# tkeskita/smoothMesh

Measured on AMD Instinct MI355X. Metric: mesh-points smoothed/sec/node (100 iters) + achieved HBM GB/s vs roofline, higher is better.
Workload: dtype f64

## Files before the change

### include/smgpu.h

```cpp
#ifndef SMGPU_H
#define SMGPU_H

#include <stddef.h>
#include <stdint.h>

#ifdef __cplusplus
extern "C" {
#endif

typedef struct smgpu_handle smgpu_handle;

typedef struct smgpu_mesh_desc {
    int32_t nPoints, nCells, nFaces, nInternalFaces;
    const double* points;
    const int32_t* faceOffsets;
    const int32_t* facePoints;
    const int32_t* owner;
    const int32_t* neighbour;
    const uint8_t* isInternalPoint;
    const uint8_t* isSmoothingSurfacePoint;
    int32_t device;
    void* stream;
    int32_t useCallerStream;
} smgpu_mesh_desc;
// ... 123 lines not shown
    void* localFlags;
} smgpu_push_desc;
int smgpu_halo_set_push(smgpu_handle* h, const smgpu_push_desc* d);
int smgpu_push_alloc(int32_t device, size_t bytes, void** ptr, void* ipcHandle64);
int smgpu_push_open(int32_t device, const void* ipcHandle64, void** ptr);
int smgpu_push_close(void* ptr);
int smgpu_push_free(void* ptr);

int smgpu_halo_set_exchange_stream(smgpu_handle* h, int32_t useExchangeStream, void* exchangeStream);
int smgpu_get_stream(smgpu_handle* h, void** stream);
int smgpu_halo_set_stats_history(smgpu_handle* h, void* history, int32_t capacity);
int smgpu_iter_begin(smgpu_handle* h);
int smgpu_iter_interior(smgpu_handle* h);
int smgpu_iter_mid(smgpu_handle* h);
int smgpu_iter_ahead(smgpu_handle* h);
int smgpu_iter_end(smgpu_handle* h);

typedef struct smgpu_layer_desc {
    int32_t nPatches;
    const int32_t* patchStart;
    const int32_t* patchSize;
    const uint8_t* patchKind;
    const uint8_t* isLayerPatch;
    double layerMaxBlendingFraction;
    double layerEdgeLength;
    double layerExpansionRatio;
    int32_t minLayers, maxLayers;
} smgpu_layer_desc;
int smgpu_set_layers(smgpu_handle* h, const smgpu_layer_desc* d, int32_t* enabled);

enum { SMGPU_LAYERS_HOPS_SWEEP = 0, SMGPU_LAYERS_NORMALS_ACCUMULATE = 1, SMGPU_LAYERS_NORMALS_FINISH = 2,
       SMGPU_LAYERS_PROPAGATE_SWEEP = 3, SMGPU_LAYERS_FINISH = 4 };
enum { SMGPU_LAYERS_F_HOPS = 0,
       SMGPU_LAYERS_F_NORMALS_COUNT = 1,
       SMGPU_LAYERS_F_NORMALS = 2 };
#define SMGPU_HALO_L_DOUBLES 14
#define SMGPU_HALO_L_LAYERS 6
int smgpu_halo_l_doubles(smgpu_handle* h, int32_t* doublesPerSlot);
int smgpu_layers_begin(smgpu_handle* h, const smgpu_layer_desc* d, int32_t* enabled, int32_t* maxIter);
int smgpu_layers_step(smgpu_handle* h, int32_t step, int32_t arg);
int smgpu_layers_shared(smgpu_handle* h, int32_t field, int32_t set, double* values);

typedef struct smgpu_boundary_desc {
    int32_t nPatches;
    const int32_t* patchStart;
    const int32_t* patchSize;
    const uint8_t* patchKind;
    const uint8_t* isSmoothingPatch;
    int32_t nInitEdgePoints;   const double* initEdgePoints;
    int32_t nInitEdges;        const int32_t* initEdges;
    int32_t nTargetEdgePoints; const double* targetEdgePoints;
    int32_t nTargetEdges;      const int32_t* targetEdges;
    int32_t nSurfacePoints;    const double* surfacePoints;
    int32_t nSurfaceTriangles; const int32_t* surfaceTriangles;
    const int32_t* isCornerPointIO;
    const int32_t* isFeatureEdgePointIO;
    double distanceTolerance;
    double internalSmoothingBlendingFraction;
} smgpu_boundary_desc;
typedef struct smgpu_boundary_info {
    int32_t enabled;
    int32_t nCornerPoints, nFeatureEdgePoints, nSmoothingSurfacePoints, nFrozenSurfacePoints;
    int32_t nTargetEdgeStrings;
} smgpu_boundary_info;
int smgpu_set_boundary_smoothing(smgpu_handle* h, const smgpu_boundary_desc* d, smgpu_boundary_info* info);
enum { SMGPU_BOUNDARY_HOPS_SWEEP = 0, SMGPU_BOUNDARY_TABLES = 1, SMGPU_BOUNDARY_NORMALS_ACCUMULATE = 2, SMGPU_BOUNDARY_NORMALS_FINISH = 3 };
enum { SMGPU_BOUNDARY_F_HOPS = 0,
       SMGPU_BOUNDARY_F_NORMALS_COUNT = 1 };
int smgpu_boundary_stats(smgpu_handle* h, double* minEdgeLength, double* boundingBox );
int smgpu_boundary_begin(smgpu_handle* h, const smgpu_boundary_desc* d, double minEdgeLengthGlobal, double perimeterGlobal,
                         smgpu_boundary_info* info);
int smgpu_boundary_step(smgpu_handle* h, int32_t step);
int smgpu_boundary_shared(smgpu_handle* h, int32_t field, int32_t set, double* values);
int smgpu_get_boundary_classification(smgpu_handle* h, int32_t* isCornerPoint, int32_t* isFeatureEdgePoint);
int smgpu_debug_edge_strings(int32_t nPoints, int32_t nEdges, const int32_t* edges, int32_t* strings, int32_t* nStrings);
int smgpu_debug_find_line(smgpu_handle* h, int32_t n, const double* segments, double* hitPoints, int32_t* hit);

int smgpu_set_device_share(smgpu_handle* h, int32_t nEngines);

int smgpu_debug_walk_mode(smgpu_handle* h, int32_t* mode, int32_t* switches, int32_t* lastCount);
#define SMGPU_TOPO_CHECKSUMS 64
int smgpu_debug_addressing_checksums(smgpu_handle* h, uint64_t* out );
int smgpu_debug_tile_checksums(smgpu_handle* h, uint64_t* out );
int smgpu_debug_halo_mode(smgpu_handle* h, int32_t* multiRole, int32_t* flagged, int32_t* fixInside);

int smgpu_debug_selftest_fpexact(int32_t device, uint64_t seed, int64_t n, int64_t* mismatches);

int smgpu_debug_get_field(smgpu_handle* h, const char* name, double* out, int64_t* n);
int smgpu_debug_get_addressing(smgpu_handle* h, const char* kind, int32_t* offsets, int32_t* values, int64_t* nnz);
int smgpu_debug_propose(smgpu_handle* h);


typedef struct smgpu_topology smgpu_topology;
int smgpu_topology_create(const smgpu_mesh_desc* desc, smgpu_topology** out);
int smgpu_topology_get(smgpu_topology* t, const char* kind, int32_t* offsets, int32_t* values, int64_t* nnz);
int smgpu_topology_num_edges(smgpu_topology* t, int32_t* nEdges);
int smgpu_topology_checksums(smgpu_topology* t, uint64_t* out );
int smgpu_topology_destroy(smgpu_topology* t);

#ifdef __cplusplus
}
#endif
#endif
```

### smoothmesh_amd/_ffi.py

```python
import ctypes as C
import os

_HERE = os.path.dirname(os.path.abspath(__file__))
LIB_PATH = os.environ.get("SMOOTHMESH_SMGPU_LIB", os.path.join(_HERE, "csrc", "libsmgpu.so"))

c_i32p = C.POINTER(C.c_int32)
c_f64p = C.POINTER(C.c_double)
c_u8p = C.POINTER(C.c_uint8)


class MeshDesc(C.Structure):
    _fields_ = [
        ("nPoints", C.c_int32), ("nCells", C.c_int32), ("nFaces", C.c_int32), ("nInternalFaces", C.c_int32),
        ("points", c_f64p), ("faceOffsets", c_i32p), ("facePoints", c_i32p), ("owner", c_i32p),
        ("neighbour", c_i32p), ("isInternalPoint", c_u8p), ("isSmoothingSurfacePoint", c_u8p),
        ("device", C.c_int32), ("stream", C.c_void_p), ("useCallerStream", C.c_int32),
    ]


class Params(C.Structure):
    _fields_ = [
        ("maxStepLength", C.c_double), ("relStepFrac", C.c_double), ("minEdgeLength", C.c_double),
        ("totalMinFreeze", C.c_int32), ("edgeAngleConstraint", C.c_int32), ("faceAngleConstraint", C.c_int32),
        ("minAngle", C.c_double), ("maxAngle", C.c_double),
# ... 75 lines not shown
        ("minFaceArea", C.c_double), ("maxFaceArea", C.c_double), ("nZeroAreaFaces", C.c_int64),
        ("maxNonOrth", C.c_double), ("avgNonOrth", C.c_double), ("nSevereNonOrth", C.c_int64), ("nErrorNonOrth", C.c_int64),
        ("maxNonOrthFace", C.c_int32),
        ("maxSkewness", C.c_double), ("nSkewFaces", C.c_int64), ("maxSkewFace", C.c_int32),
        ("nWrongOrientedFaces", C.c_int64),
        ("maxOpenness", C.c_double), ("nOpenCells", C.c_int64),
        ("maxAspectRatio", C.c_double), ("nHighAspectCells", C.c_int64),
    ]


class QualityCoupling(C.Structure):
    _fields_ = [("myRank", C.c_int32), ("nPatches", C.c_int32), ("patchStart", c_i32p), ("patchSize", c_i32p), ("neighbRank", c_i32p)]


class QualityPart(C.Structure):
    _fields_ = [("sumNonOrth" if n == "avgNonOrth" else n, t) for n, t in Quality._fields_]


SYMBOLS = {
    "smgpu_last_error": (C.c_char_p, []),
    "smgpu_version": (C.c_char_p, []),
    "smgpu_create": (C.c_int, [C.POINTER(MeshDesc), C.POINTER(C.c_void_p)]),
    "smgpu_destroy": (C.c_int, [C.c_void_p]),
    "smgpu_get_sizes": (C.c_int, [C.c_void_p, C.POINTER(Sizes)]),
    "smgpu_mesh_stats": (C.c_int, [C.c_void_p, c_f64p, c_f64p]),
    "smgpu_set_params": (C.c_int, [C.c_void_p, C.POINTER(Params)]),
    "smgpu_set_foam_variant": (C.c_int, [C.c_void_p, C.c_int32]),
    "smgpu_set_sync_variant": (C.c_int, [C.c_void_p, C.c_int32]),
    "smgpu_halo_set_push": (C.c_int, [C.c_void_p, C.POINTER(PushDesc)]),
    "smgpu_push_alloc": (C.c_int, [C.c_int32, C.c_size_t, C.POINTER(C.c_void_p), C.c_void_p]),
    "smgpu_push_open": (C.c_int, [C.c_int32, C.c_void_p, C.POINTER(C.c_void_p)]),
    "smgpu_push_close": (C.c_int, [C.c_void_p]),
    "smgpu_push_free": (C.c_int, [C.c_void_p]),
    "smgpu_set_device_share": (C.c_int, [C.c_void_p, C.c_int32]),
    "smgpu_debug_walk_mode": (C.c_int, [C.c_void_p, C.POINTER(C.c_int32), C.POINTER(C.c_int32), C.POINTER(C.c_int32)]),
    "smgpu_debug_halo_mode": (C.c_int, [C.c_void_p, C.POINTER(C.c_int32), C.POINTER(C.c_int32), C.POINTER(C.c_int32)]),
    "smgpu_debug_selftest_fpexact": (C.c_int, [C.c_int32, C.c_uint64, C.c_int64, C.POINTER(C.c_int64)]),
    "smgpu_iterate": (C.c_int, [C.c_void_p, C.c_int32, C.c_double, C.POINTER(IterStats), c_i32p]),
    "smgpu_get_points": (C.c_int, [C.c_void_p, c_f64p]),
    "smgpu_check_error": (C.c_int, [C.c_void_p]),
    "smgpu_get_near_ties": (C.c_int, [C.c_void_p, C.POINTER(C.c_int64)]),
    "smgpu_set_points": (C.c_int, [C.c_void_p, c_f64p]),
    "smgpu_enable_timing": (C.c_int, [C.c_void_p, C.c_int32]),
    "smgpu_get_counters": (C.c_int, [C.c_void_p, C.POINTER(Counters)]),
    "smgpu_reset_counters": (C.c_int, [C.c_void_p]),
    "smgpu_halo_configure": (C.c_int, [C.c_void_p, C.POINTER(HaloDesc)]),
    "smgpu_iter_begin": (C.c_int, [C.c_void_p]),
    "smgpu_iter_interior": (C.c_int, [C.c_void_p]),
    "smgpu_iter_mid": (C.c_int, [C.c_void_p]),
    "smgpu_iter_ahead": (C.c_int, [C.c_void_p]),
    "smgpu_halo_set_stats_history": (C.c_int, [C.c_void_p, C.c_void_p, C.c_int32]),
    "smgpu_set_layers": (C.c_int, [C.c_void_p, C.POINTER(LayerDesc), c_i32p]),
    "smgpu_layers_begin": (C.c_int, [C.c_void_p, C.POINTER(LayerDesc), c_i32p, c_i32p]),
    "smgpu_layers_step": (C.c_int, [C.c_void_p, C.c_int32, C.c_int32]),
    "smgpu_layers_shared": (C.c_int, [C.c_void_p, C.c_int32, C.c_int32, c_f64p]),
    "smgpu_set_boundary_smoothing": (C.c_int, [C.c_void_p, C.POINTER(BoundaryDesc), C.POINTER(BoundaryInfo)]),
    "smgpu_boundary_stats": (C.c_int, [C.c_void_p, c_f64p, c_f64p]),
    "smgpu_boundary_begin": (C.c_int, [C.c_void_p, C.POINTER(BoundaryDesc), C.c_double, C.c_double, C.POINTER(BoundaryInfo)]),
    "smgpu_boundary_step": (C.c_int, [C.c_void_p, C.c_int32]),
    "smgpu_boundary_shared": (C.c_int, [C.c_void_p, C.c_int32, C.c_int32, c_f64p]),
    "smgpu_get_boundary_classification": (C.c_int, [C.c_void_p, c_i32p, c_i32p]),
    "smgpu_debug_edge_strings": (C.c_int, [C.c_int32, C.c_int32, c_i32p, c_i32p, c_i32p]),
    "smgpu_debug_find_line": (C.c_int, [C.c_void_p, C.c_int32, c_f64p, c_f64p, c_i32p]),
    "smgpu_halo_l_doubles": (C.c_int, [C.c_void_p, c_i32p]),
    "smgpu_halo_set_exchange_stream": (C.c_int, [C.c_void_p, C.c_int32, C.c_void_p]),
    "smgpu_get_stream": (C.c_int, [C.c_void_p, C.POINTER(C.c_void_p)]),
    "smgpu_iter_end": (C.c_int, [C.c_void_p]),
    "smgpu_mesh_quality": (C.c_int, [C.c_void_p, C.POINTER(QualityParams), C.POINTER(Quality)]),
    "smgpu_quality_field": (C.c_int, [C.c_void_p, C.c_char_p, c_f64p, C.POINTER(C.c_int64)]),
    "smgpu_quality_coupled_pack": (C.c_int, [C.c_void_p, C.POINTER(QualityCoupling), C.c_void_p, C.POINTER(C.c_int64)]),
    "smgpu_quality_coupled_report": (C.c_int, [C.c_void_p, C.POINTER(QualityParams), C.c_void_p, C.POINTER(QualityPart)]),
    "smgpu_quality_coupled_field": (C.c_int, [C.c_void_p, C.c_char_p, C.c_void_p, c_f64p, C.POINTER(C.c_int64)]),
    "smgpu_quality_sets": (C.c_int, [C.c_void_p, C.POINTER(QualityParams), C.POINTER(C.c_int64), c_i32p, C.c_int64]),
    "smgpu_quality_coupled_sets": (C.c_int, [C.c_void_p, C.POINTER(QualityParams), C.c_void_p, C.POINTER(C.c_int64), c_i32p, C.c_int64]),
    "smgpu_debug_get_field": (C.c_int, [C.c_void_p, C.c_char_p, c_f64p, C.POINTER(C.c_int64)]),
    "smgpu_debug_get_addressing": (C.c_int, [C.c_void_p, C.c_char_p, c_i32p, c_i32p, C.POINTER(C.c_int64)]),
    "smgpu_debug_propose": (C.c_int, [C.c_void_p]),
    "smgpu_topology_create": (C.c_int, [C.POINTER(MeshDesc), C.POINTER(C.c_void_p)]),
    "smgpu_topology_get": (C.c_int, [C.c_void_p, C.c_char_p, c_i32p, c_i32p, C.POINTER(C.c_int64)]),
    "smgpu_topology_num_edges": (C.c_int, [C.c_void_p, c_i32p]),
    "smgpu_topology_checksums": (C.c_int, [C.c_void_p, C.POINTER(C.c_uint64)]),
    "smgpu_debug_addressing_checksums": (C.c_int, [C.c_void_p, C.POINTER(C.c_uint64)]),
    "smgpu_debug_tile_checksums": (C.c_int, [C.c_void_p, C.POINTER(C.c_uint64)]),
    "smgpu_topology_destroy": (C.c_int, [C.c_void_p]),
}

_lib = None


def lib():
    global _lib
    if _lib is None:
        if not os.path.exists(LIB_PATH):
            raise RuntimeError(
                f"{LIB_PATH} is missing: build it with `python -c 'import __graft_entry__ as g; g.build()'` "
                "or `make -C smoothmesh_amd/csrc` (hipcc --offload-arch=gfx950). There is no CPU fallback.")
        try:
            import torch
        except ImportError:
            pass
        l = C.CDLL(LIB_PATH)
        for name, (res, args) in SYMBOLS.items():
            fn = getattr(l, name)
            fn.restype = res
            fn.argtypes = args
        _lib = l
    return _lib
```

### smoothmesh_amd/csrc/kernels_tiled.hpp

```cpp
#pragma once
#include "kernels.hpp"

#ifndef SMGPU_STAGGER
#define SMGPU_STAGGER 0
#endif
__device__ __forceinline__ void staggerFirstRound(int bid, int resident) {
#if SMGPU_STAGGER
    if (bid < resident) {
        const unsigned slot = __builtin_amdgcn_s_getreg((3 << 11) | (0 << 6) | 4) & 15u;
        for (unsigned k = 0; k < slot; ++k) __builtin_amdgcn_s_sleep(SMGPU_STAGGER);
    }
#else
    (void)bid; (void)resident;
#endif
}
#ifndef SMGPU_ABLATE
#define SMGPU_ABLATE 0
#endif
namespace smgpu {

constexpr unsigned kPad = 0xFFFFu;

struct GeomTileView {
    const int* cellOrder; const int* cellBeg; const int* tpOff; const int* tpIds; const int* tfOff; const int* tfIds;
    const int* fvBase; const uint8_t* fvWidth; const uint16_t* faceVerts;
    const int* cfBase; const uint8_t* cfWidth; const uint16_t* cellFaces;
    const uint8_t* tileFlags;
    const int* meta;
    int maxPoints, maxFaces;
};
struct GeomTileMeta { int tpOff, nPts, tfOff, nFaces, fvBase, fvWidth, cellBeg, nCells, cfBase, cfWidth, flags, pad; };
constexpr int kGeomMetaInts = 12;
typedef const __attribute__((address_space(4))) int* const_int_ptr;
__device__ __forceinline__ GeomTileMeta loadTileMeta(const GeomTileView& g, int tile) {
    const_int_ptr p = (const_int_ptr)(g.meta + (size_t)kGeomMetaInts * tile);
    GeomTileMeta t;
    t.tpOff = p[0]; t.nPts = p[1]; t.tfOff = p[2]; t.nFaces = p[3]; t.fvBase = p[4]; t.fvWidth = p[5];
    t.cellBeg = p[6]; t.nCells = p[7]; t.cfBase = p[8]; t.cfWidth = p[9]; t.flags = p[10]; t.pad = 0;
    return t;
}

struct SmoothTileView {
    const int* ptOrder; const int* ptBeg; const int* tcOff; const int* tcIds; const int* tnOff; const int* tnIds;
    const uint16_t* selfLoc;
    const int* pcBase; const uint8_t* pcWidth; const uint16_t* pcEll;
    const int* ppBase; const uint8_t* ppWidth; const uint16_t* ppEll;
    const uint16_t* pairEll;
    const int* pfBase; const uint8_t* pfWidth; const uint16_t* pfEll;
    const int* meta;
    int maxCells, maxPoints, usePairShare;
};

__device__ __forceinline__ SmoothTileView pickView(bool a, const SmoothTileView& x, const SmoothTileView& y) {
    SmoothTileView v;
#define SMGPU_PICK(F) v.F = a ? x.F : y.F;
    SMGPU_PICK(ptOrder) SMGPU_PICK(ptBeg) SMGPU_PICK(tcOff) SMGPU_PICK(tcIds) SMGPU_PICK(tnOff) SMGPU_PICK(tnIds) SMGPU_PICK(selfLoc)
    SMGPU_PICK(pcBase) SMGPU_PICK(pcWidth) SMGPU_PICK(pcEll) SMGPU_PICK(ppBase) SMGPU_PICK(ppWidth) SMGPU_PICK(ppEll) SMGPU_PICK(pairEll)
    SMGPU_PICK(pfBase) SMGPU_PICK(pfWidth) SMGPU_PICK(pfEll) SMGPU_PICK(meta) SMGPU_PICK(maxCells) SMGPU_PICK(maxPoints) SMGPU_PICK(usePairShare)
#undef SMGPU_PICK
    return v;
}

struct SmoothTileMeta { int ptBeg, nPts, tcOff, nCells, tnOff, nNbrs, pcBase, pcWidth, ppBase, ppWidth, pfBase, pfWidth; };
constexpr int kSmoothMetaInts = 12;
__device__ __forceinline__ SmoothTileMeta loadTileMeta(const SmoothTileView& g, int tile) {
    const_int_ptr p = (const_int_ptr)(g.meta + (size_t)kSmoothMetaInts * tile);
    SmoothTileMeta t;
    t.ptBeg = p[0]; t.nPts = p[1]; t.tcOff = p[2]; t.nCells = p[3]; t.tnOff = p[4]; t.nNbrs = p[5];
    t.pcBase = p[6]; t.pcWidth = p[7]; t.ppBase = p[8]; t.ppWidth = p[9]; t.pfBase = p[10]; t.pfWidth = p[11];
    return t;
}

__device__ __forceinline__ int launchTile(int n, int xcdMap, int b = (int)blockIdx.x) {
    if (!xcdMap) return b;
    const int per = (n + 7) >> 3;
    const int i = (b & 7) * per + (b >> 3);
    return i < n ? i : -1;
}
__host__ __device__ inline int tileGrid(int n, int xcdMap) { return xcdMap ? ((n + 7) >> 3) << 3 : n; }

__device__ __forceinline__ V3 ldsv(const double* x, const double* y, const double* z, int i) { return v3(x[i], y[i], z[i]); }

__device__ __forceinline__ void sqrtExact4(double m0, double m1, double m2, double m3, double& a0, double& a1, double& a2, double& a3) {
    const unsigned h0 = (unsigned)__double2hiint(m0), h1 = (unsigned)__double2hiint(m1), h2 = (unsigned)__double2hiint(m2),
                   h3 = (unsigned)__double2hiint(m3);
    const unsigned lo = min(min(h0, h1), min(h2, h3)), hi = max(max(h0, h1), max(h2, h3));
    if (SMGPU_FPEXACT_FAST && __builtin_expect(lo >= ((1023u - 767u) << 20) && hi < (2047u << 20), 1)) {
        a0 = sqrtCore(m0); a1 = sqrtCore(m1); a2 = sqrtCore(m2); a3 = sqrtCore(m3);
    } else {
        a0 = sqrt(m0); a1 = sqrt(m1); a2 = sqrt(m2); a3 = sqrt(m3);
    }
}

#define SMGPU_ELL_ENTRY(J, E, BODY) { const int j = (J); const unsigned e = (E); if (e != kPad) { BODY } }
#define SMGPU_ELL_FOREACH(ROWS, W4, STRIDE, BODY)                         \
    for (int c_ = 0; c_ < (W4); ++c_) {                                   \
        const ushort4 q_ = (ROWS)[(size_t)c_ * (STRIDE)];                 \
        SMGPU_ELL_ENTRY(4 * c_ + 0, q_.x, BODY)                           \
        SMGPU_ELL_ENTRY(4 * c_ + 1, q_.y, BODY)                           \
        SMGPU_ELL_ENTRY(4 * c_ + 2, q_.z, BODY)                           \
        SMGPU_ELL_ENTRY(4 * c_ + 3, q_.w, BODY)                           \
    }

#define SMGPU_ELL_CHUNK(C, Q, BODY)                                       \
    {                                                                     \
        SMGPU_ELL_ENTRY(4 * (C) + 0, (Q).x, BODY)                         \
        SMGPU_ELL_ENTRY(4 * (C) + 1, (Q).y, BODY)                         \
        SMGPU_ELL_ENTRY(4 * (C) + 2, (Q).z, BODY)                         \
        SMGPU_ELL_ENTRY(4 * (C) + 3, (Q).w, BODY)                         \
    }
#define SMGPU_ELL_FOREACH_PRE(Q0, Q1, ROWS, W4, STRIDE, BODY)             \
    {                                                                     \
        if ((W4) > 0) SMGPU_ELL_CHUNK(0, Q0, BODY)                        \
        if ((W4) > 1) SMGPU_ELL_CHUNK(1, Q1, BODY)                        \
        for (int c_ = 2; c_ < (W4); ++c_) {                               \
            const ushort4 q_ = (ROWS)[(size_t)c_ * (STRIDE)];             \
            SMGPU_ELL_CHUNK(c_, q_, BODY)                                 \
        }                                                                 \
    }

template <int T, int ROUNDS, int STRIDE = 1>
__device__ __forceinline__ void stageRecords(const double* __restrict__ src, const int* __restrict__ ids, int n, double* x,
                                             double* y, double* z, int tid) {
    for (int base = 0; base < n; base += T * ROUNDS) {
        int id[ROUNDS];
#pragma unroll
        for (int u = 0; u < ROUNDS; ++u) {
            const int i = base + u * T + tid;
            id[u] = (i < n) ? ids[i] : -1;
        }
        V3 v[ROUNDS];
#pragma unroll
        for (int u = 0; u < ROUNDS; ++u) v[u] = (id[u] >= 0) ? ldv(src, id[u]) : v3(0, 0, 0);
#pragma unroll
        for (int u = 0; u < ROUNDS; ++u) {
            const int i = base + u * T + tid;
            if (id[u] >= 0) { x[STRIDE * i] = v[u].x; y[STRIDE * i] = v[u].y; z[STRIDE * i] = v[u].z; }
        }
    }
}

// ... 207 lines not shown
    in.mine = tid < tm.nCells;
    in.c = 0;
    in.qa = in.qb = make_ushort4(0, 0, 0, 0);
    if (in.mine) {
        in.c = g.cellOrder[ci];
        if ((tflags & 2u)) {
            const ushort4* row = reinterpret_cast<const ushort4*>(g.cellFaces + tm.cfBase) + tid;
            in.qa = row[0]; in.qb = row[T];
        }
    }
    return in;
}
template <int T, bool ORG>
__device__ __forceinline__ void geomCell(const State& s, const GeomTileView& g, const GeomLds& L, const GeomTileMeta& tm, int tid, unsigned tflags, const GeomCellIn& in,
                                         bool coh = false) {
    const double *fcx = L.fcx, *fcy = L.fcy, *fcz = L.fcz, *fax = L.fax, *fay = L.fay, *faz = L.faz;
    if (!in.mine) return;
    const int c = in.c;
    const int cw4 = tm.cfWidth >> 2;
    const ushort4* row = reinterpret_cast<const ushort4*>(g.cellFaces + tm.cfBase) + tid;
    V3 cEst = v3(0, 0, 0), ctr = v3(0, 0, 0);
    double vol = 0.0;
#define SMGPU_PYR(E, FC)                                                                                   \
    {                                                                                                      \
        const V3 fA = ldsg(fax, fay, faz, kGF * ((E) & 0x7fff));                                                   \
         \
        double pyr3Vol = dot(fA, (FC) - cEst);                                                             \
        pyr3Vol = ((E) & 0x8000) ? -pyr3Vol : pyr3Vol;                                                     \
        if (ORG) pyr3Vol = (pyr3Vol > SMGPU_VSMALL) ? pyr3Vol : SMGPU_VSMALL;    \
        const V3 pc = (3.0 / 4.0) * (FC) + (1.0 / 4.0) * cEst;                                             \
        ctr = ctr + pyr3Vol * pc;                                                                          \
        vol += pyr3Vol;                                                                                    \
    }
    if ((tflags & 2u)) {
        const ushort4 qa = in.qa, qb = in.qb;
        const unsigned e0 = qa.x, e1 = qa.y, e2 = qa.z, e3 = qa.w, e4 = qb.x, e5 = qb.y;
        const V3 c0 = ldsg(fcx, fcy, fcz, kGF * (e0 & 0x7fff)), c1 = ldsg(fcx, fcy, fcz, kGF * (e1 & 0x7fff)), c2 = ldsg(fcx, fcy, fcz, kGF * (e2 & 0x7fff)),
                 c3 = ldsg(fcx, fcy, fcz, kGF * (e3 & 0x7fff)), c4 = ldsg(fcx, fcy, fcz, kGF * (e4 & 0x7fff)), c5 = ldsg(fcx, fcy, fcz, kGF * (e5 & 0x7fff));
        cEst = cEst + c0; cEst = cEst + c1; cEst = cEst + c2; cEst = cEst + c3; cEst = cEst + c4; cEst = cEst + c5;
        cEst = divExact(cEst, 6.0);
        SMGPU_PYR(e0, c0) SMGPU_PYR(e1, c1) SMGPU_PYR(e2, c2) SMGPU_PYR(e3, c3) SMGPU_PYR(e4, c4) SMGPU_PYR(e5, c5)
    } else {
        int nFaces = 0;
        SMGPU_ELL_FOREACH(row, cw4, T, {
            cEst = cEst + ldsg(fcx, fcy, fcz, kGF * (e & 0x7fff));
            nFaces = j + 1;
        })
        cEst = divByCount(cEst, nFaces);
        SMGPU_ELL_FOREACH(row, cw4, T, {
            (void)j;
            const V3 fc = ldsg(fcx, fcy, fcz, kGF * (e & 0x7fff));
            SMGPU_PYR(e, fc)
        })
    }
#undef SMGPU_PYR
    if (fabs(vol) > SMGPU_VSMALL) ctr = divExact(ctr, vol);
    else ctr = cEst;
    if (coh) stvCoh(s.cellCtr, c, ctr); else stv(s.cellCtr, c, ctr);
}

#ifndef SMGPU_GEOM_WAVES
#define SMGPU_GEOM_WAVES 5
#endif
template <int T>
__device__ __forceinline__ void geomLoadIds(const GeomTileView& g, const GeomTileMeta& tm, int tid, int (&id)[2]) {
    const int* ids = g.tpIds + tm.tpOff;
#pragma unroll
    for (int u = 0; u < 2; ++u) { const int i = u * T + tid; id[u] = (i < tm.nPts) ? ids[i] : -1; }
}
struct GeomRows { ushort4 fq[2]; GeomCellIn cin; bool preFaces; };
template <int T, bool ORG>
__device__ __forceinline__ GeomRows geomLoadRows(const GeomTileView& g, const GeomTileMeta& tm, int tid) {
    GeomRows r;
    const unsigned tflags = (unsigned)tm.flags;
    r.preFaces = !ORG && (tflags & 1u);
#pragma unroll
    for (int u = 0; u < 2; ++u) {
        const int i = u * T + tid;
        r.fq[u] = (r.preFaces && i < tm.nFaces) ? reinterpret_cast<const ushort4*>(g.faceVerts + tm.fvBase)[i] : make_ushort4(0, 0, 0, 0);
    }
    r.cin = geomCellLoad<T>(g, tm, tid, tflags);
    return r;
}
__device__ __forceinline__ void geomLoadPoints(const State& s, const int (&id)[2], V3 (&v)[2]) {
#pragma unroll
    for (int u = 0; u < 2; ++u) v[u] = (id[u] >= 0) ? ldv(s.ptsCur, id[u]) : v3(0, 0, 0);
}
template <int T>
__device__ __forceinline__ void geomStorePoints(const State& s, const GeomTileView& g, const GeomTileMeta& tm, const GeomLds& L, const int (&id)[2],
                                                const V3 (&v)[2], int tid) {
#pragma unroll
    for (int u = 0; u < 2; ++u) {
        const int i = u * T + tid;
        if (id[u] >= 0) { L.px[kGP * i] = v[u].x; L.py[kGP * i] = v[u].y; L.pz[kGP * i] = v[u].z; }
    }
    if (tm.nPts > 2 * T)
        stageRecords<T, 2, kGP>(s.ptsCur, g.tpIds + tm.tpOff + 2 * T, tm.nPts - 2 * T, L.px + kGP * 2 * T, L.py + kGP * 2 * T, L.pz + kGP * 2 * T, tid);
}
template <int T, bool ORG>
__device__ __forceinline__ void geomFaces(const State& s, const GeomTileView& g, const GeomLds& L, const GeomTileMeta& tm, const GeomRows& r, int tid,
                                          int wantAvg, int writeFaces) {
    const unsigned tflags = (unsigned)tm.flags;
    const int nf = tm.nFaces;
#pragma unroll
    for (int u = 0; u < 2; ++u) {
        const int i = u * T + tid;
        if (i < nf) geomFace<ORG>(s, g, L, tm, i, tflags, wantAvg, writeFaces, r.preFaces, r.fq[u]);
    }
    for (int i = 2 * T + tid; i < nf; i += T) geomFace<ORG>(s, g, L, tm, i, tflags, wantAvg, writeFaces);
}

template <int T, bool ORG>
__device__ __forceinline__ void geomTileBody(const MeshView& m, const State& s, const GeomTileView& g, int wantAvg, int writeFaces, const int* tileList,
                                             int nLaunch, int xcdMap, int deferN, int deferIter, double* deferLocal, double* deferHist, int bid, bool coh = false) {
    const int stopped = s.acc->stop;
    const int li = launchTile(nLaunch, xcdMap, bid);
    if (li < 0) return;
    staggerFirstRound(bid, 256 * 4);
    if (deferN > 0 && bid == 0) { if (stopped) return; finishPartials<T>(s, deferN, deferIter, -1.0, deferLocal, deferHist); __syncthreads(); }
    extern __shared__ double lds[];
    const int tid = threadIdx.x;
    const int tile = tileList ? ((const_int_ptr)tileList)[li] : li;
    const GeomTileMeta tm = loadTileMeta(g, tile);
    const GeomLds L = geomLds(lds, tm);
    int id[2];
    geomLoadIds<T>(g, tm, tid, id);
    const GeomRows r = geomLoadRows<T, ORG>(g, tm, tid);
    V3 v[2];
    geomLoadPoints(s, id, v);
    geomStorePoints<T>(s, g, tm, L, id, v, tid);
    if (stopped) return;
    __syncthreads();
    if (SMGPU_ABLATE & 32) { if (tid < tm.nCells) stv(s.cellCtr, ((const_int_ptr)g.cellOrder)[tm.cellBeg + tid], v3(L.px[tid], 0.0, 0.0)); return; }
    geomFaces<T, ORG>(s, g, L, tm, r, tid, wantAvg, writeFaces);
    __syncthreads();
    if (SMGPU_ABLATE & 64) return;
    geomCell<T, ORG>(s, g, L, tm, tid, (unsigned)tm.flags, r.cin, coh);
}
template <int T, bool ORG>
__global__ void __launch_bounds__(T, (SMGPU_GEOM_WAVES * T) / 256) k_geom_tile(MeshView m, State s, GeomTileView g, int wantAvg, int writeFaces, const int* tileList,
                                                  int nLaunch, int xcdMap, int deferN, int deferIter, double* deferLocal,
                                                  double* deferHist) {
    geomTileBody<T, ORG>(m, s, g, wantAvg, writeFaces, tileList, nLaunch, xcdMap, deferN, deferIter, deferLocal, deferHist, (int)blockIdx.x);
}

struct SmoothLds { double *cx, *cy, *cz, *nx, *ny, *nz; };
__device__ __forceinline__ SmoothLds smoothLds(double* lds, const SmoothTileMeta& tm) {
    SmoothLds L;
    L.cx = lds;                 L.cy = L.cx + tm.nCells;  L.cz = L.cy + tm.nCells;
    L.nx = L.cz + tm.nCells;    L.ny = L.nx + tm.nNbrs;   L.nz = L.ny + tm.nNbrs;
    return L;
}
struct Top3 {
    double l1 = 0, l2 = 0, l3 = 0;
    unsigned w1 = 0xFFFFFFFFu, w2 = 0xFFFFFFFFu, w3 = 0xFFFFFFFFu;
    __device__ __forceinline__ void offer(double len, int j, unsigned e, bool take) {
        const unsigned w = ((unsigned)j << 16) | e;
        const bool b1 = take && (w1 == 0xFFFFFFFFu || len < l1);
        const bool b2 = take && !b1 && (w2 == 0xFFFFFFFFu || len < l2);
        const bool b3 = take && !b1 && !b2 && (w3 == 0xFFFFFFFFu || len < l3);
        const bool b12 = b1 || b2;
        l3 = b12 ? l2 : (b3 ? len : l3);  w3 = b12 ? w2 : (b3 ? w : w3);
        l2 = b1 ? l1 : (b2 ? len : l2);   w2 = b1 ? w1 : (b2 ? w : w2);
        l1 = b1 ? len : l1;               w1 = b1 ? w : w1;
    }
    __device__ __forceinline__ bool has2() const { return w2 != 0xFFFFFFFFu; }
    __device__ __forceinline__ bool has3() const { return w3 != 0xFFFFFFFFu; }
    __device__ __forceinline__ int k1() const { return (int)(w1 >> 16); }
    __device__ __forceinline__ int k2() const { return (int)(w2 >> 16); }
};
struct SmoothRow {
    bool mine; int p, selfL, wn4, wc4, slot;
    int peer, dst0, ndst;
    unsigned fl;
    const ushort4 *ppRow, *pcRow;
    ushort4 pp0, pp1, pc0, pc1;
    ushort4 pe0, pe1;
};
template <int T>
__device__ __forceinline__ unsigned pairBits(const SmoothTileView& g, const SmoothTileMeta& tm, const SmoothRow& R, int tid, int k) {
    if (k < 8) {
        const ushort4 q = (k & 4) ? R.pe1 : R.pe0;
        const unsigned lo = (k & 1) ? q.y : q.x, hi = (k & 1) ? q.w : q.z;
        return (k & 2) ? hi : lo;
    }
    const uint16_t* pe = g.pairEll + tm.ppBase;
    return pe[((size_t)(k >> 2) * T + tid) * 4 + (k & 3)];
}
struct SlotTabs { const int* slot; const int* peer; const int* dst0; const int* ndst; };
template <int T, bool COHC = false, int SLOTS = 1>
__device__ __forceinline__ SmoothRow smoothStage(const MeshView& m, const State& s, const SmoothTileView& g, const SmoothTileMeta& tm,
                                                 const SmoothLds& L, int tid, const SlotTabs& tb = SlotTabs{nullptr, nullptr, nullptr, nullptr}) {
    SmoothRow r;
    r.peer = -1; r.dst0 = -1; r.ndst = 0;
    r.mine = tid < tm.nPts;
    r.wn4 = tm.ppWidth >> 2; r.wc4 = tm.pcWidth >> 2;
    const int lane = r.mine ? tid : 0;
    r.ppRow = reinterpret_cast<const ushort4*>(g.ppEll + tm.ppBase) + tid;
    r.pcRow = reinterpret_cast<const ushort4*>(g.pcEll + tm.pcBase) + tid;
    const bool fast = tm.nCells <= 2 * T && tm.nNbrs <= 3 * T && r.wn4 > 0 && r.wc4 > 0;
    const ushort4 padq = make_ushort4(0xFFFF, 0xFFFF, 0xFFFF, 0xFFFF);
    if (fast) {
        const int* ic = g.tcIds + tm.tcOff;
        const int* in = g.tnIds + tm.tnOff;
        int a[2], b[3];
#pragma unroll
        for (int u = 0; u < 2; ++u) { const int i = u * T + tid; a[u] = (i < tm.nCells) ? ic[i] : -1; }
#pragma unroll
        for (int u = 0; u < 3; ++u) { const int i = u * T + tid; b[u] = (i < tm.nNbrs) ? in[i] : -1; }
        const int pi = tm.ptBeg + lane;
        const int p = g.ptOrder[pi];
        const int selfL = g.selfLoc[pi];
        const ushort4* ppl = reinterpret_cast<const ushort4*>(g.ppEll + tm.ppBase) + lane;
        const ushort4* pcl = reinterpret_cast<const ushort4*>(g.pcEll + tm.pcBase) + lane;
        const ushort4 pp0 = ppl[0], pp1 = ppl[r.wn4 > 1 ? T : 0], pc0 = pcl[0], pc1 = pcl[r.wc4 > 1 ? T : 0];
        const ushort4* pel = reinterpret_cast<const ushort4*>((g.usePairShare ? g.pairEll : g.ppEll) + tm.ppBase) + lane;
        r.pe0 = pel[0]; r.pe1 = pel[r.wn4 > 1 ? T : 0];
        int slot = -1, peer = -1, dst0 = -1, ndst = 0;
        if (SLOTS == 2) { slot = tb.slot[pi]; if (tb.peer) { peer = tb.peer[pi]; dst0 = tb.dst0[pi]; ndst = tb.ndst[pi]; } }
        V3 va[2], vb[3];
#pragma unroll
        for (int u = 0; u < 2; ++u) va[u] = (a[u] >= 0) ? (COHC ? ldvCoh(s.cellCtr, a[u]) : ldv(s.cellCtr, a[u])) : v3(0, 0, 0);
#pragma unroll
        for (int u = 0; u < 3; ++u) vb[u] = (b[u] >= 0) ? ldv(s.ptsCur, b[u]) : v3(0, 0, 0);
        const unsigned fl = m.pflags[p];
        if (SLOTS == 1) slot = s.sharedSlot ? s.sharedSlot[p] : -1;
#pragma unroll
        for (int u = 0; u < 2; ++u) { const int i = u * T + tid; if (a[u] >= 0) { L.cx[i] = va[u].x; L.cy[i] = va[u].y; L.cz[i] = va[u].z; } }
#pragma unroll
        for (int u = 0; u < 3; ++u) { const int i = u * T + tid; if (b[u] >= 0) { L.nx[i] = vb[u].x; L.ny[i] = vb[u].y; L.nz[i] = vb[u].z; } }
        r.p = r.mine ? p : 0; r.selfL = r.mine ? selfL : 0;
        r.fl = fl; r.slot = r.mine ? slot : -1; r.peer = r.mine ? peer : -1; r.dst0 = dst0; r.ndst = r.mine ? ndst : 0;
        r.pp0 = r.mine ? pp0 : padq; r.pp1 = (r.mine && r.wn4 > 1) ? pp1 : padq;
        r.pc0 = r.mine ? pc0 : padq; r.pc1 = (r.mine && r.wc4 > 1) ? pc1 : padq;
        return r;
    }
    r.p = 0; r.selfL = 0; r.fl = 0; r.slot = -1;
    r.pp0 = padq; r.pp1 = padq; r.pc0 = padq; r.pc1 = padq; r.pe0 = padq; r.pe1 = padq;
    if (r.mine) {
        if (g.usePairShare) {
            const ushort4* peRow = reinterpret_cast<const ushort4*>(g.pairEll + tm.ppBase) + tid;
            if (r.wn4 > 0) r.pe0 = peRow[0];
            if (r.wn4 > 1) r.pe1 = peRow[T];
        }
        const int pi = tm.ptBeg + tid;
        r.p = g.ptOrder[pi];
        r.selfL = g.selfLoc[pi];
        if (r.wn4 > 0) r.pp0 = r.ppRow[0];
        if (r.wn4 > 1) r.pp1 = r.ppRow[T];
        if (r.wc4 > 0) r.pc0 = r.pcRow[0];
        if (r.wc4 > 1) r.pc1 = r.pcRow[T];
        r.fl = m.pflags[r.p];
        if (SLOTS == 1) r.slot = s.sharedSlot ? s.sharedSlot[r.p] : -1;
        if (SLOTS == 2) { r.slot = tb.slot[pi]; if (tb.peer) { r.peer = tb.peer[pi]; r.dst0 = tb.dst0[pi]; r.ndst = tb.ndst[pi]; } }
    }
    if (COHC) stageRecordsCoh<T>(s.cellCtr, g.tcIds + tm.tcOff, tm.nCells, L.cx, L.cy, L.cz, tid);
    else stageRecords<T, 2>(s.cellCtr, g.tcIds + tm.tcOff, tm.nCells, L.cx, L.cy, L.cz, tid);
    stageRecords<T, 3>(s.ptsCur, g.tnIds + tm.tnOff, tm.nNbrs, L.nx, L.ny, L.nz, tid);
    return r;
}

template <bool FINAL, int T, int MODE = 0>
__device__ __forceinline__ void smoothPoint(const MeshView& m, const State& s, const Prm& prm, const SmoothTileView& g, const SmoothLds& L,
                                            const SmoothRow& R, const SmoothTileMeta& tm, int tid, double& dist, int& fcount, bool spTile = false) {
    const double *cx = L.cx, *cy = L.cy, *cz = L.cz, *nx = L.nx, *ny = L.ny, *nz = L.nz;
    const bool mine = R.mine;
    const int p = R.p, selfL = R.selfL, wn4 = R.wn4, wc4 = R.wc4;
    const ushort4 *ppRow = R.ppRow, *pcRow = R.pcRow;
    const ushort4 pp0 = R.pp0, pp1 = R.pp1, pc0 = R.pc0, pc1 = R.pc1;
    if ((SMGPU_ABLATE & 16) && !spTile) { if (mine) stv(FINAL ? s.ptsNext : s.prop, p, ldsv(nx, ny, nz, selfL)); return; }
    if (mine && !(MODE == 2 && !spTile && R.slot >= 0)) {
        const unsigned fl = R.fl;
        const bool internal = fl & PF_INTERNAL;
        const V3 cur = ldsv(nx, ny, nz, selfL);
        V3 sum = v3(0, 0, 0), r1, r2, r3;
        double m1 = 0.0, m2 = 0.0, m3 = 0.0;
        int count = 0, hc = 0;
        double shortestCur = SMGPU_GREAT;
        const int slot = (MODE == 1 || (MODE == 2 && !spTile)) ? -1 : R.slot;
        if (slot >= 0) {
            {
                const double* r = s.combA + (size_t)slot * SMGPU_HALO_A_DOUBLES;
                double w[SMGPU_HALO_A_DOUBLES];
#pragma unroll
                for (int q = 0; q < SMGPU_HALO_A_DOUBLES; ++q) w[q] = (MODE == 2 && R.peer < 0) ? ldCoh(r + q) : r[q];
                sum = v3(w[0], w[1], w[2]);
                r1 = v3(w[3], w[4], w[5]); r2 = v3(w[6], w[7], w[8]); r3 = v3(w[9], w[10], w[11]);
                const long long pk = __double_as_longlong(w[12]);
                count = (int)(pk & 0xffffffffll);
                hc = (int)(pk >> 32);
            }
            m1 = mag(r1); m2 = mag(r2); m3 = mag(r3);
            SMGPU_ELL_FOREACH_PRE(pp0, pp1, ppRow, wn4, T, {
                (void)j;
                const double len = mag(cur - ldsv(nx, ny, nz, e & 0x7fff));
                if (len < shortestCur) shortestCur = len;
            })
        } else {
            if (internal || prm.bndOn) {
                if (!(SMGPU_ABLATE & 8))
// ... 8 lines not shown
                const double len = (SMGPU_ABLATE & 1) ? magSqr(dv_) : mag(dv_);
                if (len < shortestCur) shortestCur = len;
                t3.offer(len, j, e, internal || !(e & 0x8000));
            })
            if (!t3.has2()) { s.acc->err = 1; r1 = r2 = r3 = v3(0, 0, 0); }
            else {
                r1 = ldsv(nx, ny, nz, t3.w1 & 0x7fff) - cur;
                r2 = ldsv(nx, ny, nz, t3.w2 & 0x7fff) - cur;
                r3 = !t3.has3() ? v3(SMGPU_GREAT, SMGPU_GREAT, SMGPU_GREAT) : ldsv(nx, ny, nz, t3.w3 & 0x7fff) - cur;
                m1 = t3.l1; m2 = t3.l2; m3 = !t3.has3() ? mag(r3) : t3.l3;
                if (g.usePairShare) {
                    hc = (pairBits<T>(g, tm, R, tid, t3.k1()) >> t3.k2()) & 1;
                } else {
                    const int nb = m.ppOff[p];
                    hc = shareCell(m, m.ppPt[nb + t3.k1()], m.ppPt[nb + t3.k2()]) ? 1 : 0;
                }
            }
        }
        V3 np = cur;
        if (count) np = divByCount(sum, count);
        const double blendFrac = arRatioLen(r1, r2, m1, m2, m3, hc != 0, internal);
        if (blendFrac > 0.0) {
            const V3 aCoords = cur + 0.5 * (r1 + r2);
            np = (1.0 - blendFrac) * np + blendFrac * aCoords;
        }
        {
            const V3 stepDir = np - cur;
            const double len = mag(stepDir);
            const double globalScale = (len > prm.maxStep) ? prm.maxStep / (len * prm.relStepFrac) : 1.0;
            np = cur + (prm.relStepFrac * globalScale) * stepDir;
        }
        if (prm.layersOn) np = layerTreat(s, prm, p, internal, cur, np);
        const bool deferBnd = prm.bndOn && !internal;
        if (prm.bndOn && internal) {
            const V3 stepDir = np - cur;
            const double len = mag(stepDir);
            const double globalScale = (len > prm.maxStep) ? prm.maxStep / (len * prm.relStepFrac) : 1.0;
            np = cur + (prm.relStepFrac * globalScale) * stepDir;
        }
        bool frozen = false;
        {
            double minSqr = __builtin_inf();
            if (!(SMGPU_ABLATE & 4))
            SMGPU_ELL_FOREACH_PRE(pp0, pp1, ppRow, wn4, T, {
                (void)j;
                const double t2 = magSqr(np - ldsv(nx, ny, nz, (SMGPU_ABLATE & 2) ? 0 : (e & 0x7fff)));
                if (t2 < minSqr) minSqr = t2;
            })
            const double rootMin = sqrtExact(minSqr);
            const double shortestNew = (rootMin < SMGPU_GREAT) ? rootMin : SMGPU_GREAT;
            const double shortest = (shortestNew < shortestCur) ? shortestNew : shortestCur;
            if (prm.totalMinFreeze && (shortest < prm.minEdge)) frozen = true;
            else if ((shortestNew < prm.minEdge) && (shortestNew < shortestCur)) frozen = true;
        }
        if (deferBnd) stv(s.prop, p, np);
        else if (FINAL && slot >= 0) {
            if (MODE == 2 && s.ownF) {
                stvCoh(s.prop, p, np);
                __hip_atomic_store(s.ownF + slot, frozen ? 1 : 0, __ATOMIC_RELAXED, __HIP_MEMORY_SCOPE_AGENT);
            } else stv(s.prop, p, np);
            s.frozen[p] = frozen ? 1 : 0;
            if (MODE == 2) {
                const int v = frozen ? 1 : 0;
                if (R.ndst == 1) { if (s.push.slotF) stPeer(s.push.slotF[R.dst0], v); else s.sendF[R.dst0] = v; }
                else
                    for (int k = s.sendOff[slot]; k < s.sendOff[slot + 1]; ++k) {
                        const int sl = s.sendSlots[k];
                        if (s.push.slotF) stPeer(s.push.slotF[sl], v); else s.sendF[sl] = v;
                    }
            } else if (s.inlinePackF)
                for (int k = s.sendOff[slot]; k < s.sendOff[slot + 1]; ++k) s.sendF[s.sendSlots[k]] = frozen ? 1 : 0;
        } else if (FINAL) {
            if (frozen || (!internal && !(fl & PF_SMOOTHSURF))) { np = cur; fcount = 1; }
            dist = mag(np - cur) / prm.maxStep;
            stv(s.ptsNext, p, np);
        } else {
            stv(s.prop, p, np);
            s.frozen[p] = frozen ? 1 : 0;
            if (s.stepSqr) s.stepSqr[p] = magSqr(np - cur);
        }
    }
}

template <bool FINAL, int T>
__global__ void __launch_bounds__(T) k_smooth_tile(MeshView m, State s, Prm prm, SmoothTileView g, const int* tileList,
                                                    int nLaunch, int xcdMap) {
    const int stopped = s.acc->stop;
    const int li = launchTile(nLaunch, xcdMap);
    if (li < 0) return;
    staggerFirstRound((int)blockIdx.x, 256 * 6);
    extern __shared__ double lds[];
    const int tile = tileList ? ((const_int_ptr)tileList)[li] : li, tid = threadIdx.x;
    const SmoothTileMeta tm = loadTileMeta(g, tile);
    const SmoothLds L = smoothLds(lds, tm);
    const SmoothRow R = smoothStage<T>(m, s, g, tm, L, tid);
    if (stopped) return;
    __syncthreads();
    double dist = 0.0;
    int fcount = 0;
    smoothPoint<FINAL, T>(m, s, prm, g, L, R, tm, tid, dist, fcount);
    if (FINAL) blockPublish<T>(s, dist, fcount, tile);
}

struct PackView {
    double* ownA; double* sendA;
    const int* sendOff; const int* sendSlots;
    int centroidAll;
};
template <int T, bool COHC = false, bool SP = false>
__device__ __forceinline__ void packTileBody(const MeshView& m, const State& s, const SmoothTileView& g, const PackView& pk, const int* tileList, int nLaunch,
                                             int xcdMap, int bid) {
    const int li = launchTile(nLaunch, xcdMap, bid);
    if (li < 0) return;
    extern __shared__ double lds[];
    const int tile = tileList ? ((const_int_ptr)tileList)[li] : li, tid = threadIdx.x;
    const SmoothTileMeta tm = loadTileMeta(g, tile);
    const SmoothLds L = smoothLds(lds, tm);
    const SmoothRow R = smoothStage<T, COHC, SP ? 2 : 1>(m, s, g, tm, L, tid, SlotTabs{s.spSlot, s.spPeer, s.spDst0, s.spNDst});
    __syncthreads();
    if (!R.mine) return;
    const int p = R.p;
    const int slot = R.slot;
    if (slot < 0) return;
    const double *cx = L.cx, *cy = L.cy, *cz = L.cz, *nx = L.nx, *ny = L.ny, *nz = L.nz;
    const int wn4 = R.wn4, wc4 = R.wc4;
    const ushort4 *ppRow = R.ppRow, *pcRow = R.pcRow;
    const ushort4 pp0 = R.pp0, pp1 = R.pp1, pc0 = R.pc0, pc1 = R.pc1;
    const bool internal = R.fl & PF_INTERNAL;
    const V3 cur = ldsv(nx, ny, nz, R.selfL);
    V3 sum = v3(0, 0, 0), r1, r2, r3;
    int count = 0, hc = 0;
    if (internal || pk.centroidAll) {
        SMGPU_ELL_FOREACH_PRE(pc0, pc1, pcRow, wc4, T, {
            sum = sum + ldsv(cx, cy, cz, e);
            count = j + 1;
        })
    }
    Top3 t3;
    SMGPU_ELL_FOREACH_PRE(pp0, pp1, ppRow, wn4, T, {
        const double len = mag(cur - ldsv(nx, ny, nz, e & 0x7fff));
        t3.offer(len, j, e, internal || !(e & 0x8000));
    })
    if (!t3.has2()) { s.acc->err = 1; r1 = r2 = r3 = v3(0, 0, 0); }
    else {
        r1 = ldsv(nx, ny, nz, t3.w1 & 0x7fff) - cur;
        r2 = ldsv(nx, ny, nz, t3.w2 & 0x7fff) - cur;
        r3 = !t3.has3() ? v3(SMGPU_GREAT, SMGPU_GREAT, SMGPU_GREAT) : ldsv(nx, ny, nz, t3.w3 & 0x7fff) - cur;
        if (g.usePairShare) {
            hc = (pairBits<T>(g, tm, R, tid, t3.k1()) >> t3.k2()) & 1;
        } else {
            const int nb = m.ppOff[p];
            hc = shareCell(m, m.ppPt[nb + t3.k1()], m.ppPt[nb + t3.k2()]) ? 1 : 0;
        }
    }
    double rec[SMGPU_HALO_A_DOUBLES];
    rec[0] = sum.x; rec[1] = sum.y; rec[2] = sum.z;
    rec[3] = r1.x; rec[4] = r1.y; rec[5] = r1.z;
    rec[6] = r2.x; rec[7] = r2.y; rec[8] = r2.z;
    rec[9] = r3.x; rec[10] = r3.y; rec[11] = r3.z;
    rec[12] = __longlong_as_double(((long long)hc << 32) | (long long)(unsigned int)count);
    double* o = pk.ownA + (size_t)slot * SMGPU_HALO_A_DOUBLES;
#pragma unroll
    for (int q = 0; q < SMGPU_HALO_A_DOUBLES; ++q) o[q] = rec[q];
    const int kBeg = (SP && R.ndst == 1) ? 0 : pk.sendOff[slot], kEnd = (SP && R.ndst == 1) ? 1 : pk.sendOff[slot + 1];
    for (int k = kBeg; k < kEnd; ++k) {
        const int sl = (SP && R.ndst == 1) ? R.dst0 : pk.sendSlots[k];
        if (s.push.slotA) {
            double* d = s.push.slotA[sl];
            if (((size_t)d & 8u) == 0) {
#pragma unroll
                for (int q = 0; q < 12; q += 2) stPeer2(d + q, rec[q], rec[q + 1]);
                stPeer(d + 12, rec[12]);
            } else {
                stPeer(d, rec[0]);
#pragma unroll
                for (int q = 1; q < 13; q += 2) stPeer2(d + q, rec[q], rec[q + 1]);
            }
            continue;
// ... 136 lines not shown
```

### smoothmesh_amd/csrc/smgpu.hip

```cpp
#include <hip/hip_runtime.h>
#include <hip/hip_ext.h>

#include <algorithm>
#include <chrono>
#include <future>
#include <memory>
#include <mutex>
#include <cstdio>
#include <cstring>
#include <string>
#include <vector>

#include "kernels.hpp"
#include "layers.hpp"
#include "kernels_tiled.hpp"
#include "kernels_walk.hpp"
#include "kernels_filter.hpp"
#include "kernels_boundary.hpp"
#include "kernels_quality.hpp"
#include "boundary.hpp"
#include "tiles.hpp"
#include "topology.hpp"
#include "parallel.hpp"

// ... 647 lines not shown
        rc |= devUpload(h, &m.peEdge, t.pointEdges.val);
        rc |= devUpload(h, &m.pfOff, t.pointFaces.off);
        rc |= devUpload(h, &m.pfFace, t.pointFaces.val);
        rc |= devUpload(h, &m.pfPrev, t.pfPrev);
        rc |= devUpload(h, &m.pfNext, t.pfNext);
        rc |= devUpload(h, &m.pfPrevSlot, t.pfPrevSlot);
        rc |= devUpload(h, &m.pfNextSlot, t.pfNextSlot);
        rc |= devUpload(h, &m.ringFace, t.ringFace);
        rc |= devUpload(h, &m.ringCell, t.ringCell);
        rc |= devUpload(h, &m.edgeRingOk, t.edgeRingOk);
        rc |= devUpload(h, &m.edges, t.edges);
        rc |= devUpload(h, &m.efOff, t.edgeFaces.off);
        rc |= devUpload(h, &m.efFace, t.edgeFaces.val);
        rc |= devUpload(h, &m.ecOff, t.edgeCells.off);
        rc |= devUpload(h, &m.ecCell, t.edgeCells.val);
        rc |= devUpload(h, &m.ecF0, t.ecFace0);
        rc |= devUpload(h, &m.ecF1, t.ecFace1);
    }
    rc |= devUpload(h, &m.pflags, flags);
    if (rc) return cleanupE(1);
    lapC("addressing adopted / uploaded");
    h->useTiles = envInt("SMGPU_TILES", 1) != 0;
    h->useFilter = envInt("SMGPU_FILTER", 1) != 0;
    h->xcdMap = envInt("SMGPU_XCD_MAP", 1) != 0;
    h->walkStar = envInt("SMGPU_WALK_STAR", 1) != 0;
    h->starBlocks = std::max(1, envInt("SMGPU_STAR_BLOCKS", 256 * 32));
    h->walkPack = envInt("SMGPU_WALK_PACK", 1) != 0;
    h->walkCache = envInt("SMGPU_WALK_CACHE", 1) != 0;
    h->faLists = envInt("SMGPU_FA_LISTS", 1) != 0;
    h->faSideExact = envInt("SMGPU_FA_SIDE_EXACT", 1) != 0;
    h->bndInGeom = envInt("SMGPU_BND_IN_GEOM", 1) != 0;
    { const char* fv = std::getenv("SMGPU_FOAM_VARIANT"); h->foamOrg = fv && std::string(fv) == "org"; }
    { const char* sv = std::getenv("SMGPU_SYNC_VARIANT"); h->st.ownFold = (sv && std::string(sv) == "own") ? 1 : 0; }
    if (h->useTiles) {
        h->geomT = envInt("SMGPU_GEOM_T", 256);
        h->smoothT = envInt("SMGPU_SMOOTH_T", 256);
        if (h->geomT != 64 && h->geomT != 128 && h->geomT != 256) return cleanupE(fail("SMGPU_GEOM_T must be 64, 128 or 256"));
        if (h->smoothT != 64 && h->smoothT != 128 && h->smoothT != 256) return cleanupE(fail("SMGPU_SMOOTH_T must be 64, 128 or 256"));
        const int geomCells = envInt("SMGPU_GEOM_CELLS", h->geomT / 2);
        const int capGP = envInt("SMGPU_GEOM_CAPP", std::min(6 * geomCells, 1400));
        const int capGF = envInt("SMGPU_GEOM_CAPF", std::min(4 * geomCells, 1400));
        const int capSC = envInt("SMGPU_SMOOTH_CAPC", std::min(2 * h->smoothT, 1500));
        const int capSN = envInt("SMGPU_SMOOTH_CAPN", std::min(3 * h->smoothT, 1500));
        (void)geomCells; (void)capGP; (void)capGF; (void)capSC; (void)capSN;
        std::string e2 = fSmooth.valid() ? fSmooth.get() : std::string("not built");
        std::string e1 = fGeom.valid() ? fGeom.get() : std::string("not built");
        std::string e3 = fEdge.valid() ? fEdge.get() : std::string("not built");
        if (e1 == kHostTablesPending) e1 = h->gt.buildTables(h->topo);
        std::string whyD;
        if (e2 == kHostTablesPending) e2 = downloadDeferredLists(h->topo, devTopo, h->device, whyD, 1) ? "device -> host copy of the addressing: " + whyD : h->stl.buildTables(h->topo, internalMask.data());
        if (e3 == kHostTablesPending) e3 = downloadDeferredLists(h->topo, devTopo, h->device, whyD, 2) ? "device -> host copy of the addressing: " + whyD : h->etl.buildTables(h->topo);
        if (envInt("SMGPU_VERBOSE", 0))
            std::fprintf(stderr, "[smgpu] set-up: addressing %.2f s, tile tables (3 host threads) %.2f s\n", tTopo, sinceCreate() - tTopo);
        freeOwnerNeighbour(devTopo);
        lapC("tile tasks joined");
        if (!e1.empty() || !e2.empty()) {
            h->useTiles = false;
        } else {
            GeomTileView& g = h->gv;
            SmoothTileView& v = h->sv;
            auto adoptT = [&](auto*& dst, const GeomTilesDev::Arr& a) { dst = (std::remove_reference_t<decltype(dst)>)a.p; h->allocs.push_back(a.p); h->deviceBytes += (int64_t)a.bytes; };
            if (h->gtDev.valid) {
                adoptT(g.cellOrder, h->gtDev.cellOrder); adoptT(g.cellBeg, h->gtDev.cellBeg); adoptT(g.tpIds, h->gtDev.tpIds); adoptT(g.tfIds, h->gtDev.tfIds);
                adoptT(g.faceVerts, h->gtDev.faceVerts); adoptT(g.cellFaces, h->gtDev.cellFaces); adoptT(g.meta, h->gtDev.meta);
                h->gtDev.valid = false;
            } else {
                rc |= devUpload(h, &g.cellOrder, h->gt.order);
                rc |= devUpload(h, &g.cellBeg, h->gt.cellBeg);
                rc |= devUpload(h, &g.tpIds, h->gt.tpIds);
                rc |= devUpload(h, &g.tfIds, h->gt.tfIds);
                rc |= devUpload(h, &g.faceVerts, h->gt.faceVerts);
                rc |= devUpload(h, &g.cellFaces, h->gt.cellFaces);
            }
            rc |= devUpload(h, &g.tpOff, h->gt.tpOff);
            rc |= devUpload(h, &g.tfOff, h->gt.tfOff);
            rc |= devUpload(h, &g.fvBase, h->gt.fvBase);
            rc |= devUpload(h, &g.fvWidth, h->gt.fvWidth);
            rc |= devUpload(h, &g.cfBase, h->gt.cfBase);
            rc |= devUpload(h, &g.cfWidth, h->gt.cfWidth);
            rc |= devUpload(h, &g.tileFlags, h->gt.tileFlags);
            if (!g.meta) {
                const auto& gt = h->gt;
                std::vector<int> meta((size_t)kGeomMetaInts * (size_t)gt.nTiles, 0);
                for (int t = 0; t < gt.nTiles; ++t) {
                    int* r = meta.data() + (size_t)kGeomMetaInts * t;
                    r[0] = gt.tpOff[t]; r[1] = gt.tpOff[t + 1] - gt.tpOff[t]; r[2] = gt.tfOff[t]; r[3] = gt.tfOff[t + 1] - gt.tfOff[t];
                    r[4] = gt.fvBase[t]; r[5] = gt.fvWidth[t]; r[6] = gt.cellBeg[t]; r[7] = gt.cellBeg[t + 1] - gt.cellBeg[t];
                    r[8] = gt.cfBase[t]; r[9] = gt.cfWidth[t]; r[10] = gt.tileFlags[t];
                }
                rc |= devUpload(h, &g.meta, meta);
            }
            g.maxPoints = h->gt.maxPoints; g.maxFaces = h->gt.maxFaces;
            if (h->stDev.valid) {
                auto adoptS = [&](auto*& dst, const SmoothTilesDev::Arr& a) { dst = (std::remove_reference_t<decltype(dst)>)a.p; h->allocs.push_back(a.p); h->deviceBytes += (int64_t)a.bytes; };
                adoptS(v.ptOrder, h->stDev.order); adoptS(v.ptBeg, h->stDev.ptBeg); adoptS(v.tcIds, h->stDev.tcIds); adoptS(v.tnIds, h->stDev.tnIds); adoptS(v.selfLoc, h->stDev.selfLoc);
                adoptS(v.pcEll, h->stDev.pcEll); adoptS(v.ppEll, h->stDev.ppEll); adoptS(v.pairEll, h->stDev.pairEll); adoptS(v.pfEll, h->stDev.pfEll); adoptS(v.meta, h->stDev.meta);
                h->stDev.valid = false;
            } else {
                rc |= devUpload(h, &v.ptOrder, h->stl.order);
                rc |= devUpload(h, &v.ptBeg, h->stl.ptBeg);
                rc |= devUpload(h, &v.tcIds, h->stl.tcIds);
                rc |= devUpload(h, &v.tnIds, h->stl.tnIds);
                rc |= devUpload(h, &v.selfLoc, h->stl.selfLoc);
                rc |= devUpload(h, &v.pcEll, h->stl.pcEll);
                rc |= devUpload(h, &v.ppEll, h->stl.ppEll);
                rc |= devUpload(h, &v.pairEll, h->stl.pairEll);
                rc |= devUpload(h, &v.pfEll, h->stl.pfEll);
            }
            rc |= devUpload(h, &v.tcOff, h->stl.tcOff);
            rc |= devUpload(h, &v.tnOff, h->stl.tnOff);
            rc |= devUpload(h, &v.pcBase, h->stl.pcBase);
            rc |= devUpload(h, &v.pcWidth, h->stl.pcWidth);
            rc |= devUpload(h, &v.ppBase, h->stl.ppBase);
            rc |= devUpload(h, &v.ppWidth, h->stl.ppWidth);
            rc |= devUpload(h, &v.pfBase, h->stl.pfBase);
            rc |= devUpload(h, &v.pfWidth, h->stl.pfWidth);
            if (!v.meta) {
                const auto& st = h->stl;
                std::vector<int> meta((size_t)kSmoothMetaInts * (size_t)st.nTiles, 0);
                for (int t = 0; t < st.nTiles; ++t) {
                    int* r = meta.data() + (size_t)kSmoothMetaInts * t;
                    r[0] = st.ptBeg[t]; r[1] = st.ptBeg[t + 1] - st.ptBeg[t]; r[2] = st.tcOff[t]; r[3] = st.tcOff[t + 1] - st.tcOff[t];
                    r[4] = st.tnOff[t]; r[5] = st.tnOff[t + 1] - st.tnOff[t]; r[6] = st.pcBase[t]; r[7] = st.pcWidth[t];
                    r[8] = st.ppBase[t]; r[9] = st.ppWidth[t]; r[10] = st.pfBase[t]; r[11] = st.pfWidth[t];
                }
                rc |= devUpload(h, &v.meta, meta);
            }
            v.maxCells = h->stl.maxCells; v.maxPoints = h->stl.maxPoints;
            v.usePairShare = t.maxPointPoints <= 16 ? 1 : 0;
            if (h->useFilter) {
                if (e3.empty()) {
                    EdgeTileView& ev = h->ev;
                    const size_t nGeomTf = (size_t)h->gt.tfOff.back();
                    h->avgPackedCount = nGeomTf;
                    if (h->etDev.valid) {
                        std::string why;
                        if (remapEdgeFaceIdsOnDevice(g.tfIds, (long long)nGeomTf, t.nFaces, (int*)h->etDev.tfIds.p, h->etDev.nTf, h->device, why))
                            return cleanup(fail("smgpu_create: edge tile face positions: " + why));
                        auto adoptE = [&](auto*& dst, const EdgeTilesDev::Arr& a) { dst = (std::remove_reference_t<decltype(dst)>)a.p; h->allocs.push_back(a.p); h->deviceBytes += (int64_t)a.bytes; };
                        adoptE(ev.order, h->etDev.order); adoptE(ev.edgeBeg, h->etDev.edgeBeg); adoptE(ev.tpIds, h->etDev.tpIds); adoptE(ev.tfIds, h->etDev.tfIds);
                        adoptE(ev.tcIds, h->etDev.tcIds); adoptE(ev.epLoc, h->etDev.epLoc); adoptE(ev.efEll, h->etDev.efEll); adoptE(ev.ecEll, h->etDev.ecEll);
                        adoptE(ev.meta, h->etDev.meta);
                        h->etDev.valid = false;
                    } else {
                        if (h->gt.tfIds.size() != nGeomTf) {
                            h->gt.tfIds.resize(nGeomTf);
                            if (hipMemcpy(h->gt.tfIds.data(), g.tfIds, nGeomTf * 4, hipMemcpyDeviceToHost) != hipSuccess) return cleanup(fail("smgpu_create: download of the tile face ids failed"));
                        }
                        std::vector<int32_t> facePos((size_t)t.nFaces, -1);
                        for (size_t k = 0; k < h->gt.tfIds.size(); ++k)
                            if (h->gt.tfIds[k] < 0) facePos[(size_t)(h->gt.tfIds[k] & 0x7fffffff)] = (int32_t)k;
                        for (int32_t& f : h->etl.tfIds) f = facePos[(size_t)f];
                        rc |= devUpload(h, &ev.order, h->etl.order);
                        rc |= devUpload(h, &ev.edgeBeg, h->etl.edgeBeg);
                        rc |= devUpload(h, &ev.tpIds, h->etl.tpIds);
                        rc |= devUpload(h, &ev.tfIds, h->etl.tfIds);
                        rc |= devUpload(h, &ev.tcIds, h->etl.tcIds);
                        rc |= devUpload(h, &ev.epLoc, h->etl.epLoc);
                        rc |= devUpload(h, &ev.efEll, h->etl.efEll);
                        rc |= devUpload(h, &ev.ecEll, h->etl.ecEll);
                    }
                    rc |= devUpload(h, &ev.tpOff, h->etl.tpOff);
                    rc |= devUpload(h, &ev.tfOff, h->etl.tfOff);
                    rc |= devUpload(h, &ev.tcOff, h->etl.tcOff);
                    rc |= devUpload(h, &ev.efBase, h->etl.efBase);
                    rc |= devUpload(h, &ev.ecBase, h->etl.ecBase);
                    rc |= devUpload(h, &ev.efWidth, h->etl.efWidth);
                    rc |= devUpload(h, &ev.ecWidth, h->etl.ecWidth);
                    if (!ev.meta) {
                        const auto& et = h->etl;
                        std::vector<int> meta((size_t)kEdgeMetaInts * (size_t)et.nTiles, 0);
                        for (int ti = 0; ti < et.nTiles; ++ti) {
                            int* r = meta.data() + (size_t)kEdgeMetaInts * ti;
                            r[0] = et.edgeBeg[ti]; r[1] = et.edgeBeg[ti + 1] - et.edgeBeg[ti]; r[2] = et.tpOff[ti]; r[3] = et.tpOff[ti + 1] - et.tpOff[ti];
                            r[4] = et.tfOff[ti]; r[5] = et.tfOff[ti + 1] - et.tfOff[ti]; r[6] = et.tcOff[ti]; r[7] = et.tcOff[ti + 1] - et.tcOff[ti];
                            r[8] = et.efBase[ti]; r[9] = et.efWidth[ti]; r[10] = et.ecBase[ti]; r[11] = et.ecWidth[ti];
                        }
                        rc |= devUpload(h, &ev.meta, meta);
                    }
                    ev.maxPoints = h->etl.maxPoints; ev.maxFaces = h->etl.maxFaces; ev.maxCells = h->etl.maxCells;
                    h->edgeLds = sizeof(double) * 3 * maxTileTotal(h->etl.nTiles, {&h->etl.tpOff, &h->etl.tfOff, &h->etl.tcOff});
                    h->edgeTilesOk = h->edgeLds <= 64 * 1024;
                    if (envInt("SMGPU_VERBOSE", 0))
                        std::fprintf(stderr, "[smgpu] edge tiles: n=%d LDS=%zu B (maxP %d maxF %d maxC %d)\n", h->etl.nTiles, h->edgeLds, ev.maxPoints, ev.maxFaces, ev.maxCells);
                    if (h->edgeTilesOk && envInt("SMGPU_SIDE_STREAM", sideStreamDefault(t.nPoints))) {
                        if (depInit(h)) return cleanup(1);
                        if (hipStreamCreateWithFlags(&h->side, hipStreamNonBlocking) != hipSuccess ||
                            hipEventCreateWithFlags(&h->evFork, hipEventDisableTiming) != hipSuccess ||
                            hipEventCreateWithFlags(&h->evJoin, hipEventDisableTiming) != hipSuccess)
                            return cleanup(fail("side stream creation failed"));
                    }
                }
            }
            if (rc) return cleanup(1);
            {
                size_t mx = 0;
                for (int ti = 0; ti < h->gt.nTiles; ++ti)
                    mx = std::max(mx, 3 * (size_t)(h->gt.tpOff[(size_t)ti + 1] - h->gt.tpOff[(size_t)ti]) +
                                          (size_t)(SMGPU_GEOM_AOS ? kGF : 6) * (size_t)(h->gt.tfOff[(size_t)ti + 1] - h->gt.tfOff[(size_t)ti]));
                h->geomLds = sizeof(double) * mx;
            }
            h->smoothLds = sizeof(double) * 3 * maxTileTotal(h->stl.nTiles, {&h->stl.tcOff, &h->stl.tnOff});
            if (envInt("SMGPU_VERBOSE", 0))
                std::fprintf(stderr, "[smgpu] tiles: geom T=%d n=%d LDS=%zu B (maxP %d maxF %d; staged faces x%.3f, points x%.3f of the mesh's)  smooth T=%d n=%d LDS=%zu B (maxC %d maxN %d)\n",
                             h->geomT, h->gt.nTiles, h->geomLds, g.maxPoints, g.maxFaces, (double)h->gt.tfOff.back() / std::max(1, t.nFaces),
                             (double)h->gt.tpOff.back() / std::max(1, t.nPoints), h->smoothT, h->stl.nTiles, h->smoothLds, v.maxCells, v.maxPoints);
        }
    }
    {
        const char* ea = std::getenv("SMGPU_EDGE_ANGLE");
        h->eaCoop = !(ea && std::string(ea) == "faithful");
        for (int p0 = 0; p0 < t.nPoints; p0 += kEaPointsPerBlock) {
            const int p1 = std::min(t.nPoints, p0 + kEaPointsPerBlock);
            h->eaMaxEntries = std::max(h->eaMaxEntries, t.pointEdges.off[p1] - t.pointEdges.off[p0]);
        }
        if (sizeof(double) * 9 * (size_t)h->eaMaxEntries > 60 * 1024) h->eaCoop = false;
    }
    lapC("tile tables adopted / uploaded");
    State& s = h->st;
    const size_t P = t.nPoints, C = t.nCells, F = t.nFaces, E = t.nEdges;
    rc |= devAlloc(h, &h->bufA, 3 * P);
    rc |= devAlloc(h, &h->bufB, 3 * P);
    rc |= devAlloc(h, &s.prop, 3 * P);
    rc |= devAlloc(h, &h->dStepSqr, P + 4);
    rc |= devAlloc(h, &s.fCtr, 3 * F);
    rc |= devAlloc(h, &s.fArea, 3 * F);
    s.avgPacked = (h->useTiles && h->edgeTilesOk && h->avgPackedCount) ? 1 : 0;
    rc |= devAlloc(h, &s.fAvg, 3 * (s.avgPacked ? h->avgPackedCount : F));
    rc |= devAlloc(h, &s.cellCtr, 3 * C);
    rc |= devAlloc(h, &s.frozen, P);
    rc |= devAlloc(h, &s.edgeMin, E);
    rc |= devAlloc(h, &s.edgeMax, E);
    rc |= devAlloc(h, &s.ptMin, P);
    rc |= devAlloc(h, &s.ptMax, P);
    rc |= devAlloc(h, &s.faActive, P + 16);
    rc |= devAlloc(h, &h->dFaMaybe, P + 16);
    rc |= devAlloc(h, &s.faEdgeList, E);
    rc |= devAlloc(h, &s.faPointList, P);
    rc |= devAlloc(h, &h->dEaMaybe, P);
    rc |= devAlloc(h, &s.faS, P);
    rc |= devAlloc(h, &s.faN, t.pointPoints.size());
    rc |= devAlloc(h, &s.walkStack, P + 64);
    rc |= devAlloc(h, &s.acc, 1);
    rc |= devAlloc(h, &s.nearTotal, 4);
    {
        const size_t nPart = (size_t)std::max(gridFor(t.nPoints), h->useTiles ? h->stl.nTiles : 0) + 2 * (size_t)gridFor(t.nPoints) + 1;
        rc |= devAlloc(h, &s.blkMax, nPart);
        rc |= devAlloc(h, &s.blkCnt, nPart);
    }
    if (rc) return cleanup(1);
    lapC("work arrays allocated");
    if (hipMemset(s.acc, 0, sizeof(Accum)) != hipSuccess) return cleanup(fail("hipMemset failed"));
    if (hipMemsetAsync(s.nearTotal, 0, 4 * sizeof(unsigned long long), h->stream) != hipSuccess) return cleanup(fail("hipMemset failed"));
    if (hipMemset(s.frozen, 0, P) != hipSuccess) return cleanup(fail("hipMemset failed"));
    if (hipMemcpy(h->bufA, d->points, 3 * P * sizeof(double), hipMemcpyHostToDevice) != hipSuccess)
        return cleanup(fail("upload of points failed"));
    if (hipMemcpy(s.prop, h->bufA, 3 * P * sizeof(double), hipMemcpyDeviceToDevice) != hipSuccess)
        return cleanup(fail("upload of points failed"));
    lapC("points uploaded");
    s.ptsCur = h->bufA;
    s.ptsNext = h->bufB;
    s.stats = nullptr;
    s.sharedSlot = nullptr;
    s.combA = nullptr;
    {
        void* dp = nullptr;
        if (hipHostMalloc((void**)&h->nActiveHost, 64, hipHostMallocMapped) == hipSuccess &&
            hipHostGetDevicePointer(&dp, h->nActiveHost, 0) == hipSuccess) {
            *(volatile int*)h->nActiveHost = -1;
            s.nActiveHost = (int*)dp;
        } else {
            (void)hipGetLastError();
            if (h->nActiveHost) (void)hipHostFree(h->nActiveHost);
            h->nActiveHost = nullptr;
            s.nActiveHost = nullptr;
        }
    }
    computeAlgoBytes(h);
    if (fEdge.valid()) fEdge.wait();
    freeOwnerNeighbour(devTopo);
    h->devLists.owner = h->devLists.neighbour = DeviceTopologyArrays::Arr();
    if (envInt("SMGPU_VERBOSE", 0)) std::fprintf(stderr, "[smgpu] set-up: total %.2f s\n", sinceCreate());
    *out = h;
    return 0;
}
// ... 105 lines not shown
    for (long i = blockIdx.x * (long)blockDim.x + threadIdx.x; i < n; i += (long)gridDim.x * blockDim.x) {
        const double x = selftestArg(seed, i, 0), y = selftestArg(seed, i, 1), z = selftestArg(seed, i, 2), w = selftestArg(seed, i, 3);
        if (!sameBits(sqrtExact(x), sqrt(x))) ++mine;
        double a0, a1, a2, a3;
        sqrtExact4(fabs(x), fabs(y), z, fabs(w), a0, a1, a2, a3);
        if (!sameBits(a0, sqrt(fabs(x))) || !sameBits(a1, sqrt(fabs(y))) || !sameBits(a2, sqrt(z)) || !sameBits(a3, sqrt(fabs(w)))) ++mine;
        const V3 q = divExact(v3(x, y, z), w);
        if (!sameBits(q.x, x / w) || !sameBits(q.y, y / w) || !sameBits(q.z, z / w)) ++mine;
        const V3 q6 = divExact(v3(x, y, z), 6.0);
        if (!sameBits(q6.x, x / 6.0) || !sameBits(q6.y, y / 6.0) || !sameBits(q6.z, z / 6.0)) ++mine;
    }
    if (mine) atomicAdd(bad, mine);
}
}

int smgpu_debug_selftest_fpexact(int32_t device, uint64_t seed, int64_t n, int64_t* mismatches) {
    if (!mismatches || n < 0) return fail("smgpu_debug_selftest_fpexact: bad arguments");
    if (hipSetDevice(device) != hipSuccess) return fail("smgpu_debug_selftest_fpexact: hipSetDevice failed");
    unsigned long long* d = nullptr;
    if (hipMalloc(&d, sizeof(*d)) != hipSuccess) return fail("smgpu_debug_selftest_fpexact: hipMalloc failed");
    unsigned long long host = 0;
    bool ok = hipMemset(d, 0, sizeof(*d)) == hipSuccess;
    if (ok) {
        hipLaunchKernelGGL(smgpu::k_selftest_fpexact, dim3(2048), dim3(256), 0, 0, seed, (long)n, d);
        ok = hipGetLastError() == hipSuccess && hipMemcpy(&host, d, sizeof(host), hipMemcpyDeviceToHost) == hipSuccess;
    }
    (void)hipFree(d);
    if (!ok) return fail("smgpu_debug_selftest_fpexact: launch failed");
    *mismatches = (int64_t)host;
    return 0;
}

int smgpu_set_foam_variant(smgpu_handle* h, int32_t variant) {
    if (!h) return fail("null handle");
    if (variant != SMGPU_FOAM_COM && variant != SMGPU_FOAM_ORG) return fail("smgpu_set_foam_variant: unknown variant");
    h->foamOrg = variant == SMGPU_FOAM_ORG;
    h->qEpoch++;
    h->geomAheadDone = false;
    return 0;
}

int smgpu_set_sync_variant(smgpu_handle* h, int32_t variant) {
    if (!h) return fail("null handle");
    if (variant != SMGPU_SYNC_MASTER && variant != SMGPU_SYNC_OWN) return fail("smgpu_set_sync_variant: unknown variant");
    h->st.ownFold = variant == SMGPU_SYNC_OWN ? 1 : 0;
    return 0;
}

int smgpu_set_params(smgpu_handle* h, const smgpu_params* p) {
    if (!h || !p) return fail("null argument");
    if (!(p->maxStepLength > 0.0)) return fail("maxStepLength must be > 0");
    h->prm = *p;
    h->prmSet = true;
    h->walkMode = -1;
    h->walkSwitches = 0;
    h->walkDecisions = 0;
    if (h->nActiveHost) *(volatile int*)h->nActiveHost = -1;
    h->geomAheadDone = false;
    computeAlgoBytes(h);
    return 0;
}

extern "C++" {
template <typename K>
static void ensureDynLds(K kernel, int device, size_t bytes) {
    static std::mutex mu;
    static size_t have[64] = {0};
    if (bytes <= 64 * 1024 || device < 0 || device >= 64) return;
    std::lock_guard<std::mutex> lock(mu);
    if (have[device] >= bytes) return;
    if (hipFuncSetAttribute((const void*)kernel, hipFuncAttributeMaxDynamicSharedMemorySize, (int)bytes) == hipSuccess) have[device] = bytes;
    else (void)hipGetLastError();
}
template <int T, bool ORG>
static void launchGeomTileAs(smgpu_handle* h, const MeshView& m, const State& s, int wantAvg, const int* tileList, int nTiles, hipEvent_t evA, hipEvent_t evB,
                             bool withBndPre) {
    if (withBndPre) {
        const int nNormal = (h->bv.nB + T - 1) / T, nFeat = (h->bv.nFeat + (T / 64) - 1) / (T / 64);
        const int nBnd = ((nNormal + nFeat + 7) / 8) * 8;
        ensureDynLds(k_geom_tile_bnd<T, ORG>, h->device, h->geomLds);
        hipExtLaunchKernelGGL((k_geom_tile_bnd<T, ORG>), dim3(nBnd + tileGrid(nTiles, h->xcdMap)), dim3(T), (uint32_t)h->geomLds, h->stream, evA, evB, 0, m, s, h->gv,
                              wantAvg, h->writeFaces ? 1 : 0, tileList, nTiles, h->xcdMap, h->deferN, h->deferIter, h->deferLocal, h->deferHist, h->bv, nBnd, nNormal);
    } else {
        ensureDynLds(k_geom_tile<T, ORG>, h->device, h->geomLds);
        hipExtLaunchKernelGGL((k_geom_tile<T, ORG>), dim3(tileGrid(nTiles, h->xcdMap)), dim3(T), (uint32_t)h->geomLds, h->stream, evA, evB, 0, m, s, h->gv, wantAvg,
                              h->writeFaces ? 1 : 0, tileList, nTiles, h->xcdMap, h->deferN, h->deferIter, h->deferLocal, h->deferHist);
    }
    h->deferN = 0;
    h->deferLocal = h->deferHist = nullptr;
}
template <int T>
static void launchGeomTile(smgpu_handle* h, const MeshView& m, const State& s, int wantAvg, const int* tileList, int nTiles, hipEvent_t evA, hipEvent_t evB,
                           bool withBndPre) {
    if (h->foamOrg) launchGeomTileAs<T, true>(h, m, s, wantAvg, tileList, nTiles, evA, evB, withBndPre);
    else launchGeomTileAs<T, false>(h, m, s, wantAvg, tileList, nTiles, evA, evB, withBndPre);
}
template <bool FINAL, int T>
static void launchSmoothTile(smgpu_handle* h, const MeshView& m, const State& s, const Prm& prm, const int* tileList, int nTiles, hipEvent_t evA, hipEvent_t evB) {
    ensureDynLds(k_smooth_tile<FINAL, T>, h->device, h->smoothLds);
    hipExtLaunchKernelGGL((k_smooth_tile<FINAL, T>), dim3(tileGrid(nTiles, h->xcdMap)), dim3(T), (uint32_t)h->smoothLds, h->stream, evA, evB, 0, m, s, prm, h->sv,
                          tileList, nTiles, h->xcdMap);
}
template <bool FINAL>
static int launchBndFix(smgpu_handle* h, int partialBase) {
    if (h->bv.nB == 0) return 0;
    return launchK(h, K_BND, [&] {
        hipLaunchKernelGGL(k_bnd_fix<FINAL>, dim3(gridFor(2 * (int64_t)h->bv.nB)), dim3(kBlock), 0, h->stream, h->mv, h->st, makePrm(h), h->bv, partialBase);
    });
}
static int launchBndPre(smgpu_handle* h, const MeshView& m, const State& s, hipStream_t stream) {
    if (h->bv.nB == 0) return 0;
    return launchK(h, K_BND, [&] {
        hipLaunchKernelGGL(k_bnd_normals, dim3(gridFor(h->bv.nB)), dim3(kBlock), 0, stream, m, s, h->bv);
        if (h->bv.nFeat) hipLaunchKernelGGL(k_bnd_feature, dim3(h->bv.nFeat), dim3(64), 0, stream, m, s, h->bv);
    }, stream);
}
static int runBndPre(smgpu_handle* h) {
    if (h->bndOn && h->bndInGeom && h->useTiles && h->bv.nB > 0) return 0;
    if (!h->bndOn || !h->bndSide || h->bndPreInFlight || h->timing) return 0;
    if (depSignal(h, DEP_BND_FORK, h->stream, h->evBndFork) || depWait(h, DEP_BND_FORK, h->bndSide, h->evBndFork)) return 1;
    if (launchBndPre(h, h->mv, h->st, h->bndSide)) return 1;
    if (depSignal(h, DEP_BND_JOIN, h->bndSide, h->evBndJoin)) return 1;
    h->bndPreInFlight = true;
    return 0;
}
template <bool FINAL>
static int runSmooth(smgpu_handle* h, const MeshView& m, const State& s, const Prm& prm, const int* tileList = nullptr, int nList = 0) {
    const int kid = FINAL ? K_SMOOTH_FINAL : K_SMOOTH_PROP;
    const bool withBnd = h->bndOn && !h->haloOn;
    if (withBnd) {
        if (h->bndPreDone) h->bndPreDone = false;
        else if (h->bndPreInFlight) {
            if (depWait(h, DEP_BND_JOIN, h->stream, h->evBndJoin)) return 1;
            h->bndPreInFlight = false;
        } else if (launchBndPre(h, m, s, h->stream)) return 1;
    }
    if (h->useTiles) {
        const int nT = tileList ? nList : h->stl.nTiles;
        if (nT == 0) return 0;
        if (launchKDispatch(h, kid, [&](hipEvent_t evA, hipEvent_t evB) {
                if (h->smoothT == 64) launchSmoothTile<FINAL, 64>(h, m, s, prm, tileList, nT, evA, evB);
                else if (h->smoothT == 128) launchSmoothTile<FINAL, 128>(h, m, s, prm, tileList, nT, evA, evB);
                else launchSmoothTile<FINAL, 256>(h, m, s, prm, tileList, nT, evA, evB);
            })) return 1;
    } else if (launchK(h, kid, [&] { hipLaunchKernelGGL(k_smooth<FINAL>, dim3(gridFor(m.nPoints)), dim3(kBlock), 0, h->stream, m, s, prm); })) return 1;
    if (withBnd) {
        const int base = h->useTiles ? h->stl.nTiles : gridFor(m.nPoints);
        return launchK(h, K_BND, [&] { hipLaunchKernelGGL(k_bnd_fix<FINAL>, dim3(gridFor(2 * (int64_t)h->bv.nB)), dim3(kBlock), 0, h->stream, m, s, prm, h->bv, base); });
    }
    return 0;
}

}

static int runGeometry(smgpu_handle* h, const int* tileList = nullptr, int nList = 0, bool fromNext = false, bool withBndPre = false) {
    const MeshView& m = h->mv;
    State s = h->st;
    if (fromNext) s.ptsCur = h->st.ptsNext;
    const int wantAvg = h->prm.faceAngleConstraint ? 1 : 0;
    if (h->useTiles) {
        const int nT = tileList ? nList : h->gt.nTiles;
        if (nT == 0) return 0;
        const bool bnd = withBndPre && h->bndOn && h->bndInGeom && !fromNext && h->bv.nB > 0 && !h->bndPreInFlight && !h->bndPreDone;
        if (bnd) h->bndPreDone = true;
        return launchKDispatch(h, K_GEOM_TILE, [&](hipEvent_t evA, hipEvent_t evB) {
            if (h->geomT == 64) launchGeomTile<64>(h, m, s, wantAvg, tileList, nT, evA, evB, bnd);
            else if (h->geomT == 128) launchGeomTile<128>(h, m, s, wantAvg, tileList, nT, evA, evB, bnd);
            else launchGeomTile<256>(h, m, s, wantAvg, tileList, nT, evA, evB, bnd);
        });
    }
    if (launchK(h, K_FACE_GEOM, [&] { hipLaunchKernelGGL(k_face_geom, dim3(gridFor(m.nFaces)), dim3(kBlock), 0, h->stream, m, s, wantAvg, h->foamOrg ? 1 : 0); })) return 1;
    if (launchK(h, K_CELL_CENTRES, [&] { hipLaunchKernelGGL(k_cell_centres, dim3(gridFor(m.nCells)), dim3(kBlock), 0, h->stream, m, s, h->foamOrg ? 1 : 0); })) return 1;
    return 0;
}

static int ensureWalkBuffers(smgpu_handle* h) {
    if (h->walkAlloc) return 0;
    const Topology& t = h->topo;
    if (envInt("SMGPU_WALK_MEMO_STATS", 0) && !SMGPU_WALK_MEMO) return fail("SMGPU_WALK_MEMO_STATS needs a build with -DSMGPU_WALK_MEMO=1 (make HIPFLAGS+=-DSMGPU_WALK_MEMO=1)");
    if (envInt("SMGPU_WALK_MEMO_STATS", 0) && !h->dWalkMemo) {
        if (devAlloc(h, &h->dWalkMemo, (size_t)t.nPoints + 2)) return 1;
// ... 2065 lines not shown
        HIP_OK(hipStreamSynchronize(h->stream));
        const bool tagged = (bsrc == st.faActive);
        for (int64_t i = 0; i < cnt; ++i) out[i] = tagged ? (tmp[(size_t)i] == st.faGen ? 1.0 : 0.0) : (double)tmp[(size_t)i];
    }
    return 0;
}

static int topoGet(const Topology& t, const char* kind, int32_t* offsets, int32_t* values, int64_t* nnz) {
    const std::string s(kind);
    const std::vector<int32_t>* off = nullptr;
    const std::vector<int32_t>* val = nullptr;
    if (s == "pointCells") { off = &t.pointCells.off; val = &t.pointCells.val; }
    else if (s == "pointPoints") { off = &t.pointEdges.off; val = &t.pointPoints; }
    else if (s == "pointEdges") { off = &t.pointEdges.off; val = &t.pointEdges.val; }
    else if (s == "pointFaces") { off = &t.pointFaces.off; val = &t.pointFaces.val; }
    else if (s == "pointFacePrev") { off = &t.pointFaces.off; val = &t.pfPrev; }
    else if (s == "pointFaceNext") { off = &t.pointFaces.off; val = &t.pfNext; }
    else if (s == "edgeFaces") { off = &t.edgeFaces.off; val = &t.edgeFaces.val; }
    else if (s == "edgeCells") { off = &t.edgeCells.off; val = &t.edgeCells.val; }
    else if (s == "cellFacesGeom") { off = &t.cellFacesGeom.off; val = &t.cellFacesGeom.val; }
    else if (s == "edges") { val = &t.edges; }
    else return fail("unknown addressing " + s);
    *nnz = (int64_t)val->size();
    if (offsets && off) std::memcpy(offsets, off->data(), sizeof(int32_t) * off->size());
    if (values) std::memcpy(values, val->data(), sizeof(int32_t) * val->size());
    return 0;
}

static uint64_t fnv1a(const void* p, size_t n, uint64_t hh = 1469598103934665603ull) {
    const unsigned char* b = (const unsigned char*)p;
    for (size_t i = 0; i < n; ++i) { hh ^= b[i]; hh *= 1099511628211ull; }
    return hh;
}
static void topoChecksums(const Topology& t, uint64_t* out) {
    int k = 0;
    const int32_t sizes[9] = {t.nPoints, t.nCells, t.nFaces, t.nInternalFaces, t.nEdges, t.maxFaceSize, t.maxEdgeFaces, t.maxPointCells, t.maxPointPoints};
    out[k++] = fnv1a(sizes, sizeof(sizes));
    auto add = [&](const auto& v) { out[k++] = fnv1a(v.data(), v.size() * sizeof(v[0])) ^ (uint64_t)v.size(); };
    add(t.facePoints.off); add(t.facePoints.val); add(t.owner); add(t.neighbour);
    add(t.cellFacesGeom.off); add(t.cellFacesGeom.val);
    add(t.pointFaces.off); add(t.pointFaces.val); add(t.pfPrev); add(t.pfNext); add(t.pfPrevSlot); add(t.pfNextSlot);
    add(t.pointCells.off); add(t.pointCells.val);
    add(t.edges); add(t.pointEdges.off); add(t.pointEdges.val); add(t.pointPoints);
    add(t.edgeFaces.off); add(t.edgeFaces.val); add(t.edgeCells.off); add(t.edgeCells.val); add(t.ecFace0); add(t.ecFace1);
    add(t.ringFace); add(t.ringCell); add(t.edgeRingOk);
    while (k < SMGPU_TOPO_CHECKSUMS) out[k++] = 0;
}
int smgpu_debug_tile_checksums(smgpu_handle* h, uint64_t* out) {
    if (!h || !out) return fail("null argument");
    for (int i = 0; i < SMGPU_TOPO_CHECKSUMS; ++i) out[i] = 0;
    if (!h->useTiles) return 0;
    HIP_OK(hipSetDevice(h->device));
    const GeomTiles& gt = h->gt;
    const int nT = gt.nTiles;
    int k = 0;
    auto host = [&](const auto& v) { out[k++] = fnv1a(v.data(), v.size() * sizeof(v[0])) ^ (uint64_t)v.size(); };
    auto dev = [&](const void* p, size_t bytes) -> int {
        std::vector<unsigned char> buf(bytes);
        if (bytes) HIP_OK(hipMemcpy(buf.data(), p, bytes, hipMemcpyDeviceToHost));
        out[k++] = fnv1a(buf.data(), bytes) ^ (uint64_t)bytes;
        return 0;
    };
    host(gt.cellBeg); host(gt.tpOff); host(gt.tfOff); host(gt.fvBase); host(gt.fvWidth); host(gt.cfBase); host(gt.cfWidth); host(gt.tileFlags);
    const int32_t mx[2] = {gt.maxPoints, gt.maxFaces};
    out[k++] = fnv1a(mx, sizeof(mx));
    const size_t nTp = (size_t)gt.tpOff.back(), nTf = (size_t)gt.tfOff.back();
    const size_t nFv = nT ? (size_t)gt.fvBase[(size_t)nT - 1] + (size_t)(gt.tfOff[(size_t)nT] - gt.tfOff[(size_t)nT - 1]) * gt.fvWidth[(size_t)nT - 1] : 0;
    const size_t nCf = nT ? (size_t)gt.cfBase[(size_t)nT - 1] + (size_t)gt.cfWidth[(size_t)nT - 1] * (size_t)gt.threads : 0;
    if (dev(h->gv.cellOrder, (size_t)h->mv.nCells * 4) || dev(h->gv.tpIds, nTp * 4) || dev(h->gv.tfIds, nTf * 4) || dev(h->gv.faceVerts, nFv * 2) ||
        dev(h->gv.cellFaces, nCf * 2) || dev(h->gv.meta, (size_t)nT * kGeomMetaInts * 4)) return 1;
    {
        const SmoothTiles& st = h->stl;
        const int nS = st.nTiles;
        host(st.ptBeg); host(st.tcOff); host(st.tnOff); host(st.pcBase); host(st.pcWidth); host(st.ppBase); host(st.ppWidth); host(st.pfBase); host(st.pfWidth);
        const int32_t mxS[2] = {st.maxCells, st.maxPoints};
        out[k++] = fnv1a(mxS, sizeof(mxS));
        const size_t nPc = nS ? (size_t)st.pcBase[(size_t)nS - 1] + (size_t)st.pcWidth[(size_t)nS - 1] * (size_t)st.threads : 0;
        const size_t nPp = nS ? (size_t)st.ppBase[(size_t)nS - 1] + (size_t)st.ppWidth[(size_t)nS - 1] * (size_t)st.threads : 0;
        const size_t nPfE = nS ? (size_t)st.pfBase[(size_t)nS - 1] + (size_t)st.pfWidth[(size_t)nS - 1] * (size_t)st.threads : 0;
        if (dev(h->sv.ptOrder, (size_t)h->mv.nPoints * 4) || dev(h->sv.tcIds, (size_t)st.tcOff.back() * 4) || dev(h->sv.tnIds, (size_t)st.tnOff.back() * 4) ||
            dev(h->sv.selfLoc, (size_t)h->mv.nPoints * 2) || dev(h->sv.pcEll, nPc * 2) || dev(h->sv.ppEll, nPp * 2) || dev(h->sv.pairEll, nPp * 2) || dev(h->sv.pfEll, nPfE * 2) ||
            dev(h->sv.meta, (size_t)nS * kSmoothMetaInts * 4)) return 1;
    }
    if (h->useFilter && h->ev.meta) {
        const EdgeTiles& et = h->etl;
        const int nE = et.nTiles;
        host(et.tpOff); host(et.tfOff); host(et.tcOff); host(et.efBase); host(et.ecBase); host(et.efWidth); host(et.ecWidth);
        const int32_t mxE[3] = {et.maxPoints, et.maxFaces, et.maxCells};
        out[k++] = fnv1a(mxE, sizeof(mxE));
        const size_t nEf = nE ? (size_t)et.efBase[(size_t)nE - 1] + (size_t)et.efWidth[(size_t)nE - 1] * (size_t)et.threads : 0;
        const size_t nEc = nE ? (size_t)et.ecBase[(size_t)nE - 1] + (size_t)et.ecWidth[(size_t)nE - 1] * (size_t)et.threads : 0;
        if (dev(h->ev.order, (size_t)h->mv.nEdges * 4) || dev(h->ev.edgeBeg, ((size_t)nE + 1) * 4) || dev(h->ev.tpIds, (size_t)et.tpOff.back() * 4) ||
            dev(h->ev.tfIds, (size_t)et.tfOff.back() * 4) || dev(h->ev.tcIds, (size_t)et.tcOff.back() * 4) || dev(h->ev.epLoc, (size_t)h->mv.nEdges * 4) ||
            dev(h->ev.efEll, nEf * 2) || dev(h->ev.ecEll, nEc * 2) || dev(h->ev.meta, (size_t)nE * kEdgeMetaInts * 4)) return 1;
    }
    return 0;
}

int smgpu_debug_addressing_checksums(smgpu_handle* h, uint64_t* out) {
    if (!h || !out) return fail("null argument");
    if (ensureHostLists(h, 3)) return 1;
    topoChecksums(h->topo, out);
    return 0;
}

int smgpu_debug_get_addressing(smgpu_handle* h, const char* kind, int32_t* offsets, int32_t* values, int64_t* nnz) {
    if (!h || !kind || !nnz) return fail("null argument");
    if (ensureHostLists(h, 1)) return 1;
    return topoGet(h->topo, kind, offsets, values, nnz);
}

struct smgpu_topology { Topology t; };

int smgpu_topology_create(const smgpu_mesh_desc* d, smgpu_topology** out) {
    if (!d || !out) return fail("null argument");
    smgpu_topology* t = new smgpu_topology();
    const std::string terr = t->t.build(d->nPoints, d->nCells, d->nFaces, d->nInternalFaces, d->faceOffsets, d->facePoints,
                                        d->owner, d->neighbour);
    if (!terr.empty()) { delete t; *out = nullptr; return fail("smgpu_topology_create: " + terr); }
    *out = t;
    return 0;
}
int smgpu_topology_get(smgpu_topology* t, const char* kind, int32_t* offsets, int32_t* values, int64_t* nnz) {
    if (!t || !kind || !nnz) return fail("null argument");
    return topoGet(t->t, kind, offsets, values, nnz);
}
int smgpu_topology_checksums(smgpu_topology* t, uint64_t* out) {
    if (!t || !out) return fail("null argument");
    topoChecksums(t->t, out);
    return 0;
}
int smgpu_topology_num_edges(smgpu_topology* t, int32_t* nEdges) {
    if (!t || !nEdges) return fail("null argument");
    *nEdges = t->t.nEdges;
    return 0;
}
int smgpu_topology_destroy(smgpu_topology* t) { delete t; return 0; }

}
```

### smoothmesh_amd/csrc/tiles.cpp

```cpp
#include "tiles.hpp"
#include "parallel.hpp"

#include <algorithm>
#include <chrono>
#include <cstdio>
#include <cstdlib>

namespace smgpu {

namespace {
struct PhaseTimer {
    const char* who;
    bool on;
    std::chrono::steady_clock::time_point t;
    explicit PhaseTimer(const char* w) : who(w), on(std::getenv("SMGPU_VERBOSE") && std::atoi(std::getenv("SMGPU_VERBOSE")) >= 2), t(std::chrono::steady_clock::now()) {}
    void lap(const char* what) {
        const auto now = std::chrono::steady_clock::now();
        if (on) std::fprintf(stderr, "[smgpu] %s tiles: %-18s %.2f s   (done at +%.3f s)\n", who, what, std::chrono::duration<double>(now - t).count(), setupClock());
        t = now;
    }
};
}


static inline int32_t roundUp4(int32_t v) { return v <= 4 ? 4 : (v + 3) & ~3; }

static inline uint64_t spread21(uint64_t v) {
    v &= 0x1fffff;
    v = (v | v << 32) & 0x1f00000000ffffull;
    v = (v | v << 16) & 0x1f0000ff0000ffull;
    v = (v | v << 8) & 0x100f00f00f00f00full;
    v = (v | v << 4) & 0x10c30c30c30c30c3ull;
    v = (v | v << 2) & 0x1249249249249249ull;
    return v;
}

static std::vector<int32_t> mortonOrder(int32_t n, const double* xyz) {
    double lo[3] = {1e300, 1e300, 1e300}, hi[3] = {-1e300, -1e300, -1e300};
    {
        const int parts = rangeParts(n);
        std::vector<double> plo(3 * (size_t)parts, 1e300), phi(3 * (size_t)parts, -1e300);
        parallelRanges(n, parts, [&](int part, int64_t b, int64_t e) {
            double l[3] = {1e300, 1e300, 1e300}, h[3] = {-1e300, -1e300, -1e300};
            for (int64_t i = b; i < e; ++i)
                for (int a = 0; a < 3; ++a) { l[a] = std::min(l[a], xyz[3 * (size_t)i + a]); h[a] = std::max(h[a], xyz[3 * (size_t)i + a]); }
            for (int a = 0; a < 3; ++a) { plo[3 * (size_t)part + a] = l[a]; phi[3 * (size_t)part + a] = h[a]; }
        });
        for (int part = 0; part < parts; ++part)
            for (int a = 0; a < 3; ++a) { lo[a] = std::min(lo[a], plo[3 * (size_t)part + a]); hi[a] = std::max(hi[a], phi[3 * (size_t)part + a]); }
    }
    double ext = 0.0;
    for (int a = 0; a < 3; ++a) ext = std::max(ext, hi[a] - lo[a]);
    const double scale = ext > 0.0 ? 2097151.0 / ext : 0.0;
    std::vector<std::pair<uint64_t, int32_t>> key((size_t)n);
    parallelRanges(n, rangeParts(n), [&](int, int64_t b, int64_t e) {
        for (int64_t i = b; i < e; ++i) {
            uint64_t k = 0;
            for (int a = 0; a < 3; ++a) k |= spread21((uint64_t)((xyz[3 * (size_t)i + a] - lo[a]) * scale)) << a;
            key[(size_t)i] = {k, (int32_t)i};
        }
    });
    if (rangeParts(n) > 1) {
        const int shift = 55;
        std::vector<size_t> cnt(257, 0);
        for (int32_t i = 0; i < n; ++i) ++cnt[(size_t)(key[(size_t)i].first >> shift) + 1];
        for (int bkt = 0; bkt < 256; ++bkt) cnt[(size_t)bkt + 1] += cnt[(size_t)bkt];
        std::vector<std::pair<uint64_t, int32_t>> tmp((size_t)n);
        {
            std::vector<size_t> cur(cnt.begin(), cnt.end() - 1);
            for (int32_t i = 0; i < n; ++i) tmp[cur[(size_t)(key[(size_t)i].first >> shift)]++] = key[(size_t)i];
        }
        key.swap(tmp);
        std::vector<std::pair<uint64_t, int32_t>>().swap(tmp);
        parallelRanges(256, (int)std::min<unsigned>(hostThreads(), 256u), [&](int, int64_t b, int64_t e) {
            for (int64_t bkt = b; bkt < e; ++bkt) std::sort(key.begin() + (ptrdiff_t)cnt[(size_t)bkt], key.begin() + (ptrdiff_t)cnt[(size_t)bkt + 1]);
        });
    } else std::sort(key.begin(), key.end());
    std::vector<int32_t> order((size_t)n);
    for (int32_t i = 0; i < n; ++i) order[(size_t)i] = key[(size_t)i].second;
    return order;
}

std::vector<int32_t> mortonOrderOf(int32_t n, const double* xyz) { return mortonOrder(n, xyz); }

static std::vector<int32_t> naturalOrder(int32_t n) {
    std::vector<int32_t> o((size_t)n);
    for (int32_t i = 0; i < n; ++i) o[(size_t)i] = i;
    return o;
}
// ... 545 lines not shown
        std::string err;
    };
    const int parts = rangeParts(nTiles, 64);
    std::vector<Part> P((size_t)parts);
    const int32_t threadsL = threads;
    parallelRanges(nTiles, parts, [&](int part, int64_t tb, int64_t te) {
        Part& o = P[(size_t)part];
        std::vector<int32_t> pts, fcs, cls;
        for (int32_t ti = (int32_t)tb; ti < (int32_t)te; ++ti) {
            pts.clear(); fcs.clear(); cls.clear();
            const int32_t eb = edgeBeg[ti], ee = edgeBeg[ti + 1];
            int32_t wf = 0, wc = 0;
            for (int32_t ei = eb; ei < ee; ++ei) {
                const int32_t e = order[(size_t)ei];
                wf = std::max(wf, ef.off[e + 1] - ef.off[e]);
                wc = std::max(wc, ec.off[e + 1] - ec.off[e]);
                pts.push_back(t.edges[2 * e]); pts.push_back(t.edges[2 * e + 1]);
                for (int32_t k = ef.off[e]; k < ef.off[e + 1]; ++k) fcs.push_back(ef.val[k]);
                for (int32_t k = ec.off[e]; k < ec.off[e + 1]; ++k) cls.push_back(ec.val[k]);
            }
            std::sort(pts.begin(), pts.end()); pts.erase(std::unique(pts.begin(), pts.end()), pts.end());
            std::sort(fcs.begin(), fcs.end()); fcs.erase(std::unique(fcs.begin(), fcs.end()), fcs.end());
            std::sort(cls.begin(), cls.end()); cls.erase(std::unique(cls.begin(), cls.end()), cls.end());
            wf = roundUp4(wf); wc = roundUp4(wc);
            if (pts.size() > 32766 || fcs.size() > 32766 || cls.size() > 32766 || wf > 252 || wc > 252) {
                o.err = "tile too large for the 15-bit local index tables";
                return;
            }
            auto loc = [](const std::vector<int32_t>& v, int32_t x) { return (int32_t)(std::lower_bound(v.begin(), v.end(), x) - v.begin()); };
            o.tpIds.insert(o.tpIds.end(), pts.begin(), pts.end()); o.nP.push_back((int32_t)pts.size());
            o.tfIds.insert(o.tfIds.end(), fcs.begin(), fcs.end()); o.nF.push_back((int32_t)fcs.size());
            o.tcIds.insert(o.tcIds.end(), cls.begin(), cls.end()); o.nC.push_back((int32_t)cls.size());
            o.efBase.push_back((int32_t)o.efEll.size()); o.efWidth.push_back((uint8_t)wf);
            o.ecBase.push_back((int32_t)o.ecEll.size()); o.ecWidth.push_back((uint8_t)wc);
            const size_t fb = o.efEll.size(), cb = o.ecEll.size();
            o.efEll.resize(fb + (size_t)wf * threadsL, kEllPad);
            o.ecEll.resize(cb + (size_t)wc * threadsL, kEllPad);
            for (int32_t ei = eb; ei < ee; ++ei) {
                const int32_t e = order[(size_t)ei], tl = ei - eb;
                epLoc[2 * (size_t)ei] = (uint16_t)loc(pts, t.edges[2 * e]);
                epLoc[2 * (size_t)ei + 1] = (uint16_t)loc(pts, t.edges[2 * e + 1]);
                if (!t.edgeRingOk[(size_t)e]) continue;
                for (int32_t k = ef.off[e], j = 0; k < ef.off[e + 1]; ++k, ++j)
                    o.efEll[fb + ((size_t)(j / 4) * threadsL + tl) * 4 + (j % 4)] = (uint16_t)loc(fcs, t.ringFace[k]);
                for (int32_t k = ec.off[e], j = 0; k < ec.off[e + 1]; ++k, ++j)
                    o.ecEll[cb + ((size_t)(j / 4) * threadsL + tl) * 4 + (j % 4)] = (uint16_t)loc(cls, t.ringCell[k]);
            }
            o.maxPoints = std::max(o.maxPoints, (int32_t)pts.size());
            o.maxFaces = std::max(o.maxFaces, (int32_t)fcs.size());
            o.maxCells = std::max(o.maxCells, (int32_t)cls.size());
        }
    });
    tpOff.assign(1, 0); tfOff.assign(1, 0); tcOff.assign(1, 0);
    efBase.clear(); ecBase.clear(); efWidth.clear(); ecWidth.clear();
    size_t efTotal = 0, ecTotal = 0;
    for (Part& o : P) {
        if (!o.err.empty()) return o.err;
        for (int32_t n : o.nP) tpOff.push_back(tpOff.back() + n);
        for (int32_t n : o.nF) tfOff.push_back(tfOff.back() + n);
        for (int32_t n : o.nC) tcOff.push_back(tcOff.back() + n);
        for (int32_t b : o.efBase) efBase.push_back((int32_t)(efTotal + (size_t)b));
        for (int32_t b : o.ecBase) ecBase.push_back((int32_t)(ecTotal + (size_t)b));
        efWidth.insert(efWidth.end(), o.efWidth.begin(), o.efWidth.end());
        ecWidth.insert(ecWidth.end(), o.ecWidth.begin(), o.ecWidth.end());
        efTotal += o.efEll.size(); ecTotal += o.ecEll.size();
        maxPoints = std::max(maxPoints, o.maxPoints);
        maxFaces = std::max(maxFaces, o.maxFaces);
        maxCells = std::max(maxCells, o.maxCells);
    }
    if (efTotal > 0x7fffffffu || ecTotal > 0x7fffffffu) return "tile tables exceed int32 addressing";
    {
        std::vector<std::vector<int32_t>> a, b, c;
        std::vector<std::vector<uint16_t>> d, e;
        for (Part& o : P) {
            a.push_back(std::move(o.tpIds)); b.push_back(std::move(o.tfIds)); c.push_back(std::move(o.tcIds));
            d.push_back(std::move(o.efEll)); e.push_back(std::move(o.ecEll));
        }
        concatParts(tpIds, a); concatParts(tfIds, b); concatParts(tcIds, c); concatParts(efEll, d); concatParts(ecEll, e);
    }
    tm.lap("tables");
    return "";
}

}
```

### smoothmesh_amd/csrc/tiles.hpp

```cpp
#pragma once
#include <cstdint>
#include <string>
#include <vector>

#include "topology.hpp"

namespace smgpu {

constexpr uint16_t kEllPad = 0xFFFF;

std::vector<int32_t> mortonOrderOf(int32_t n, const double* xyz);

struct GeomTiles {
    int32_t nTiles = 0, threads = 0;
    std::vector<int32_t> cellBeg;
    std::vector<int32_t> tpOff;
    std::vector<int32_t> tpIds;
    std::vector<int32_t> tfOff;
    std::vector<int32_t> tfIds;
    std::vector<int32_t> fvBase;
    std::vector<uint8_t> fvWidth;
    std::vector<uint16_t> faceVerts;
    std::vector<int32_t> cfBase;
    std::vector<uint8_t> cfWidth;
    std::vector<uint16_t> cellFaces;
    std::vector<uint8_t> tileFlags;
    int32_t maxPoints = 0, maxFaces = 0;
    std::vector<int32_t> order;
    std::string build(const Topology& t, const double* points, bool morton, int32_t threads, int32_t capCells,
                      int32_t capPoints, int32_t capFaces, int32_t capWeighted = 0x7fffffff, int32_t faceWeight = 7);
    std::string buildBoundaries(const Topology& t, const double* points, bool morton, int32_t threads, int32_t capCells,
                                int32_t capPoints, int32_t capFaces, int32_t capWeighted = 0x7fffffff, int32_t faceWeight = 7,
                                const std::vector<int32_t>* cellOrder = nullptr);
    std::string buildTables(const Topology& t);
};
struct GeomTilesDev {
    struct Arr { void* p = nullptr; size_t bytes = 0; };
    Arr cellOrder, cellBeg, tpIds, tfIds, faceVerts, cellFaces, meta;
    bool valid = false;
};
struct DeviceTopologyArrays;
int cellMortonOrderOnDevice(const DeviceTopologyArrays& td, int32_t nCells, int32_t nPoints, const double* points, int device, std::vector<int32_t>& order, std::string& why);
int buildGeomTablesOnDevice(GeomTiles& gt, const DeviceTopologyArrays& td, int32_t nCells, int device, GeomTilesDev& out, std::string& why);

struct SmoothTiles {
    int32_t nTiles = 0, threads = 0;
    std::vector<int32_t> ptBeg;
    std::vector<int32_t> tcOff;
    std::vector<int32_t> tcIds;
    std::vector<int32_t> tnOff;
    std::vector<int32_t> tnIds;
    std::vector<uint16_t> selfLoc;
    std::vector<int32_t> pcBase;
    std::vector<uint8_t> pcWidth;
    std::vector<uint16_t> pcEll;
    std::vector<int32_t> ppBase;
    std::vector<uint8_t> ppWidth;
    std::vector<uint16_t> ppEll;
    std::vector<uint16_t> pairEll;
    std::vector<int32_t> pfBase;
    std::vector<uint8_t> pfWidth;
    std::vector<uint16_t> pfEll;
    int32_t maxCells = 0, maxPoints = 0;
    std::vector<int32_t> order;
    std::string build(const Topology& t, const double* points, const uint8_t* isInternal, bool morton, int32_t threads,
                      int32_t capCells, int32_t capPoints, const std::vector<int32_t>* pointOrder = nullptr,
                      const std::vector<int32_t>* subset = nullptr, int32_t capTotal = 0x7fffffff);
    std::string buildBoundaries(const Topology& t, const double* points, bool morton, int32_t threads, int32_t capCells, int32_t capPoints,
                                const std::vector<int32_t>* pointOrder = nullptr, const std::vector<int32_t>* subset = nullptr, int32_t capTotal = 0x7fffffff);
    std::string buildTables(const Topology& t, const uint8_t* isInternal, bool subset = false);
};
struct SmoothTilesDev {
    struct Arr { void* p = nullptr; size_t bytes = 0; };
    Arr order, ptBeg, tcIds, tnIds, selfLoc, pcEll, ppEll, pairEll, pfEll, meta;
    bool valid = false;
};
struct CornerChains { int* chPrev = nullptr; int* chNext = nullptr; int* bad = nullptr; int* big = nullptr; void* stream = nullptr; int32_t nPoints = 0; bool started = false; };
int startCornerChains(const DeviceTopologyArrays& td, int32_t nPoints, int device, CornerChains& c, std::string& why);
void releaseCornerChains(CornerChains& c);
int buildSmoothTablesOnDevice(SmoothTiles& st, const DeviceTopologyArrays& td, int32_t nPoints, int32_t maxPointPoints, const uint8_t* isInternal, int device,
                              SmoothTilesDev& out, std::string& why, CornerChains* chains = nullptr);

struct EdgeTiles {
    int32_t nTiles = 0, threads = 0;
    std::vector<int32_t> order;
    std::vector<int32_t> edgeBeg;
    std::vector<int32_t> tpOff, tpIds, tfOff, tfIds, tcOff, tcIds;
// ... 22 lines not shown
```

### smoothmesh_amd/csrc/tiles_dev.hip

```cpp
#include <hip/hip_runtime.h>

#include <cstring>

#include <rocprim/device/device_radix_sort.hpp>
#include <rocprim/device/device_scan.hpp>

#include <algorithm>
#include <chrono>
#include <cstdio>
#include <cstdlib>
#include <string>
#include <vector>

#include "tiles.hpp"

namespace smgpu {

namespace {

constexpr int kT = 256;
constexpr int kBuf = 4096;
constexpr int kPadKey = 0x7fffffff;
typedef unsigned long long u64;

// ... 711 lines not shown
    if (!tcIds || !tnIds || !meta || !selfLoc || !pcEll || !ppEll || !pairEll || !pfEll) { why = "device allocation failed"; return 2; }
    TL_OK(hipMemsetAsync(pcEll, 0xFF, (size_t)nPc * 2, sm));
    TL_OK(hipMemsetAsync(ppEll, 0xFF, (size_t)nPp * 2, sm));
    TL_OK(hipMemsetAsync(pfEll, 0xFF, (size_t)nPfE * 2, sm));
    TL_OK(hipMemsetAsync(pairEll, 0, (size_t)nPp * 2, sm));
    TL_OK(hipMemsetAsync(selfLoc, 0, (size_t)nPos * 2, sm));
    hipLaunchKernelGGL(k_tl_smooth<true>, dim3(nT), dim3(kT), 0, sm, in, sz,
                       SmoothOut{offsD, offsD + S, offsD + 2 * S, offsD + 3 * S, offsD + 4 * S, tcIds, tnIds, selfLoc, pcEll, ppEll, pairEll, pfEll, meta});
    std::vector<int> hC((size_t)nT), hN((size_t)nT), hWc((size_t)nT), hWn((size_t)nT), hWf((size_t)nT);
    TL_OK(hipMemcpyAsync(hC.data(), nCl, (size_t)nT * 4, hipMemcpyDeviceToHost, sm));
    TL_OK(hipMemcpyAsync(hN.data(), nPt, (size_t)nT * 4, hipMemcpyDeviceToHost, sm));
    TL_OK(hipMemcpyAsync(hWc.data(), wc, (size_t)nT * 4, hipMemcpyDeviceToHost, sm));
    TL_OK(hipMemcpyAsync(hWn.data(), wn, (size_t)nT * 4, hipMemcpyDeviceToHost, sm));
    TL_OK(hipMemcpyAsync(hWf.data(), wf, (size_t)nT * 4, hipMemcpyDeviceToHost, sm));
    TL_OK(hipStreamSynchronize(sm));
    TL_OK(hipGetLastError());
    st.tcOff.resize(S); st.tnOff.resize(S);
    st.pcBase.resize((size_t)nT); st.ppBase.resize((size_t)nT); st.pfBase.resize((size_t)nT); st.pcWidth.resize((size_t)nT); st.ppWidth.resize((size_t)nT); st.pfWidth.resize((size_t)nT);
    st.maxCells = st.maxPoints = 0;
    for (size_t i = 0; i < S; ++i) { st.tcOff[i] = (int32_t)offs[i]; st.tnOff[i] = (int32_t)offs[S + i]; }
    for (int i = 0; i < nT; ++i) {
        st.pcBase[(size_t)i] = (int32_t)offs[2 * S + i]; st.ppBase[(size_t)i] = (int32_t)offs[3 * S + i]; st.pfBase[(size_t)i] = (int32_t)offs[4 * S + i];
        st.pcWidth[(size_t)i] = (uint8_t)hWc[(size_t)i]; st.ppWidth[(size_t)i] = (uint8_t)hWn[(size_t)i]; st.pfWidth[(size_t)i] = (uint8_t)hWf[(size_t)i];
        st.maxCells = std::max(st.maxCells, hC[(size_t)i]); st.maxPoints = std::max(st.maxPoints, hN[(size_t)i]);
    }
    st.tcIds.clear(); st.tnIds.clear(); st.selfLoc.clear(); st.pcEll.clear(); st.ppEll.clear(); st.pairEll.clear(); st.pfEll.clear();
    auto give = [&](SmoothTilesDev::Arr& a, void* p, size_t bytes) { a.p = p; a.bytes = std::max<size_t>(bytes, 1); D.release(p); };
    give(out.order, dOrder, (size_t)nPos * 4); give(out.ptBeg, dBeg, S * 4); give(out.tcIds, tcIds, (size_t)nTc * 4); give(out.tnIds, tnIds, (size_t)nTn * 4);
    give(out.selfLoc, selfLoc, (size_t)nPos * 2); give(out.pcEll, pcEll, (size_t)nPc * 2); give(out.ppEll, ppEll, (size_t)nPp * 2); give(out.pairEll, pairEll, (size_t)nPp * 2);
    give(out.pfEll, pfEll, (size_t)nPfE * 2); give(out.meta, meta, 12 * (size_t)nT * 4);
    out.valid = true;
    return 0;
}

int cellMortonOrderOnDevice(const DeviceTopologyArrays& td, int32_t nCells, int32_t nPoints, const double* points, int device, std::vector<int32_t>& order, std::string& why) {
    if (!td.valid || nCells <= 0 || nPoints <= 0) return 1;
    TL_OK(hipSetDevice(device));
    hipStream_t st = nullptr;
    TL_OK(hipStreamCreateWithFlags(&st, hipStreamNonBlocking));
    struct StreamGuard { hipStream_t s; ~StreamGuard() { (void)hipStreamDestroy(s); } } guard{st};
    const int nB = (nCells + kT - 1) / kT;
    DevBuf D;
    double *dPts = D.get<double>(3 * (size_t)nPoints), *cc = D.get<double>(3 * (size_t)nCells), *part = D.get<double>(6 * (size_t)nB);
    u64 *kA = D.get<u64>((size_t)nCells), *kB = D.get<u64>((size_t)nCells);
    int *iA = D.get<int>((size_t)nCells), *iB = D.get<int>((size_t)nCells);
    if (!dPts || !cc || !part || !kA || !kB || !iA || !iB) { why = "device allocation failed"; return 2; }
    TL_OK(hipMemcpyAsync(dPts, points, 3 * (size_t)nPoints * 8, hipMemcpyHostToDevice, st));
    hipLaunchKernelGGL(k_tl_cellAvg, dim3(nB), dim3(kT), 0, st, nCells, (const int*)td.cfOff.p, (const int*)td.cfVal.p, (const int*)td.faceOff.p, (const int*)td.facePts.p, dPts, cc, part);
    std::vector<double> hp(6 * (size_t)nB);
    TL_OK(hipMemcpyAsync(hp.data(), part, hp.size() * 8, hipMemcpyDeviceToHost, st));
    TL_OK(hipStreamSynchronize(st));
    double lo[3] = {1e300, 1e300, 1e300}, hi[3] = {-1e300, -1e300, -1e300};
    for (int b = 0; b < nB; ++b)
        for (int a = 0; a < 3; ++a) { lo[a] = std::min(lo[a], hp[6 * (size_t)b + a]); hi[a] = std::max(hi[a], hp[6 * (size_t)b + 3 + a]); }
    double ext = 0.0;
    for (int a = 0; a < 3; ++a) ext = std::max(ext, hi[a] - lo[a]);
    const double scale = ext > 0.0 ? 2097151.0 / ext : 0.0;
    hipLaunchKernelGGL(k_tl_mortonKeys, dim3(nB), dim3(kT), 0, st, nCells, cc, lo[0], lo[1], lo[2], scale, kA, iA);
    size_t tempBytes = 0;
    (void)rocprim::radix_sort_pairs(nullptr, tempBytes, kA, kB, iA, iB, (size_t)nCells, 0, 63, st);
    void* temp = D.get<char>(tempBytes + 256);
    if (!temp) { why = "device allocation failed"; return 2; }
    TL_OK(rocprim::radix_sort_pairs(temp, tempBytes, kA, kB, iA, iB, (size_t)nCells, 0, 63, st));
    order.resize((size_t)nCells);
    TL_OK(hipMemcpyAsync(order.data(), iB, (size_t)nCells * 4, hipMemcpyDeviceToHost, st));
    TL_OK(hipStreamSynchronize(st));
    TL_OK(hipGetLastError());
    return 0;
}

int remapEdgeFaceIdsOnDevice(const int* geomTfIds, long long nGeomTf, int32_t nFaces, int* edgeTfIds, long long nEdgeTf, int device, std::string& why) {
    TL_OK(hipSetDevice(device));
    int* facePos = nullptr;
    TL_OK(hipMalloc((void**)&facePos, std::max<size_t>((size_t)nFaces, 1) * 4));
    struct Free { int* p; ~Free() { (void)hipFree(p); } } guard{facePos};
    TL_OK(hipMemset(facePos, 0xFF, (size_t)nFaces * 4));
    hipLaunchKernelGGL(k_tl_facePos, dim3((unsigned)((nGeomTf + kT - 1) / kT)), dim3(kT), 0, nullptr, nGeomTf, geomTfIds, facePos);
    hipLaunchKernelGGL(k_tl_remap, dim3((unsigned)((nEdgeTf + kT - 1) / kT)), dim3(kT), 0, nullptr, nEdgeTf, edgeTfIds, facePos);
    TL_OK(hipDeviceSynchronize());
    TL_OK(hipGetLastError());
    return 0;
}

}
```

### smoothmesh_amd/engine.py

```python
import ctypes as C
from dataclasses import dataclass
from typing import Optional

import numpy as np

from . import _ffi
from .mesh import PolyMesh


class SmgpuError(RuntimeError):
    """A non-zero status from the library (the reference would FatalError/abort here)."""


@dataclass
class SmoothParams:
    maxStepLength: float
    minEdgeLength: float
    relStepFrac: float = 0.5
    totalMinFreeze: bool = False
    edgeAngleConstraint: bool = True
    faceAngleConstraint: bool = True
    minAngle: float = 35.0
    maxAngle: float = 160.0

# ... 68 lines not shown
    kinds = {"processor": 1, "empty": 2}
    start = np.array([p.startFace for p in mesh.patches], np.int32)
    size = np.array([p.nFaces for p in mesh.patches], np.int32)
    kind = np.array([kinds.get(p.type, 0) for p in mesh.patches], np.uint8)
    sel = np.array([any((q.fullmatch(p.name) is not None) if hasattr(q, "fullmatch") else (q == p.name) for q in pats)
                    for p in mesh.patches], np.uint8)
    return start, size, kind, sel


def default_params(meshMinEdgeLength: float, **over) -> SmoothParams:
    minEdge = over.pop("minEdgeLength", 0.5 * meshMinEdgeLength)
    maxStep = over.pop("maxStepLength", 0.3 * minEdge)
    return SmoothParams(maxStepLength=maxStep, minEdgeLength=minEdge, **over)


def _p(a, t):
    return a.ctypes.data_as(t)


def make_desc(mesh: PolyMesh, isInternalPoint, isSmoothingSurfacePoint, device=0, stream=None):
    keep = dict(
        pts=np.ascontiguousarray(mesh.points, dtype=np.float64),
        fo=mesh.faceOffsets, fp=mesh.facePoints, ow=mesh.owner, ne=mesh.neighbour,
        ip=np.ascontiguousarray(isInternalPoint, dtype=np.uint8),
        sp=None if isSmoothingSurfacePoint is None else np.ascontiguousarray(isSmoothingSurfacePoint, dtype=np.uint8),
    )
    d = _ffi.MeshDesc()
    d.nPoints, d.nCells, d.nFaces, d.nInternalFaces = mesh.nPoints, mesh.nCells, mesh.nFaces, mesh.nInternalFaces
    d.points = _p(keep["pts"], _ffi.c_f64p)
    d.faceOffsets = _p(keep["fo"], _ffi.c_i32p)
    d.facePoints = _p(keep["fp"], _ffi.c_i32p)
    d.owner = _p(keep["ow"], _ffi.c_i32p)
    d.neighbour = _p(keep["ne"], _ffi.c_i32p)
    d.isInternalPoint = _p(keep["ip"], _ffi.c_u8p)
    d.isSmoothingSurfacePoint = _p(keep["sp"], _ffi.c_u8p) if keep["sp"] is not None else None
    d.device = device
    d.stream = stream if stream else None
    d.useCallerStream = 0 if stream is None else 1
    return d, keep


TOPO_ARRAYS = ["sizes and maxima", "facePoints.off", "facePoints.val", "owner", "neighbour", "cellFacesGeom.off", "cellFacesGeom.val",
               "pointFaces.off", "pointFaces.val", "pfPrev", "pfNext", "pfPrevSlot", "pfNextSlot", "pointCells.off", "pointCells.val",
               "edges", "pointEdges.off", "pointEdges.val", "pointPoints", "edgeFaces.off", "edgeFaces.val", "edgeCells.off", "edgeCells.val",
               "ecFace0", "ecFace1", "ringFace", "ringCell", "edgeRingOk"]


class HostTopology:

    def __init__(self, mesh: PolyMesh):
        self._lib = _ffi.lib()
        d, self._keep = make_desc(mesh, np.ones(mesh.nPoints, np.uint8), None)
        self._h = C.c_void_p()
        if self._lib.smgpu_topology_create(C.byref(d), C.byref(self._h)):
            raise SmgpuError(self._lib.smgpu_last_error().decode())

    def addressing(self, kind):
        nnz = C.c_int64()
        k = kind.encode()
        if self._lib.smgpu_topology_get(self._h, k, None, None, C.byref(nnz)):
            raise SmgpuError(self._lib.smgpu_last_error().decode())
        vals = np.empty(nnz.value, np.int32)
        if kind == "edges":
            self._lib.smgpu_topology_get(self._h, k, None, _p(vals, _ffi.c_i32p), C.byref(nnz))
            return None, vals.reshape(-1, 2)
        rows = {"pointCells": "P", "pointPoints": "P", "pointEdges": "P", "pointFaces": "P", "pointFacePrev": "P",
                "pointFaceNext": "P", "edgeFaces": "E", "edgeCells": "E", "cellFacesGeom": "C"}[kind]
        n = {"P": self._keep["pts"].shape[0], "E": self.num_edges(), "C": int(self._keep["ow"].max()) + 1}[rows]
        off = np.empty(n + 1, np.int32)
        self._lib.smgpu_topology_get(self._h, k, _p(off, _ffi.c_i32p), _p(vals, _ffi.c_i32p), C.byref(nnz))
        return off, vals

    def num_edges(self):
        n = C.c_int32()
        self._lib.smgpu_topology_num_edges(self._h, C.byref(n))
        return n.value

    def checksums(self):
        out = (C.c_uint64 * 64)()
        if self._lib.smgpu_topology_checksums(self._h, out):
            raise SmgpuError(self._lib.smgpu_last_error().decode())
        return [int(x) for x in out][:len(TOPO_ARRAYS)]

    def close(self):
        if self._h:
            self._lib.smgpu_topology_destroy(self._h)
            self._h = C.c_void_p()

    def __del__(self):
        try:
            self.close()
        except Exception:
            pass


class SmoothEngine:
    def __init__(self, mesh: PolyMesh, isInternalPoint=None, isSmoothingSurfacePoint=None, device=0, stream=None):
        self._lib = _ffi.lib()
        self.mesh = mesh
        if isInternalPoint is None:
            isInternalPoint = mesh.find_internal_points()
        if isSmoothingSurfacePoint is None:
            isSmoothingSurfacePoint = mesh.smoothing_surface_points()
        self.isInternalPoint = np.ascontiguousarray(isInternalPoint, dtype=np.uint8)
        d, keep = make_desc(mesh, self.isInternalPoint, isSmoothingSurfacePoint, device, stream)
        self._h = C.c_void_p()
        self._check(self._lib.smgpu_create(C.byref(d), C.byref(self._h)))
        self.nPoints = mesh.nPoints
        self._keepalive = []

    def _check(self, rc):
        if rc:
            raise SmgpuError(self._lib.smgpu_last_error().decode())

    def close(self):
        if getattr(self, "_h", None):
            self._lib.smgpu_destroy(self._h)
            self._h = C.c_void_p()

    def __del__(self):
        try:
            self.close()
        except Exception:
            pass

    def sizes(self):
        s = _ffi.Sizes()
        self._check(self._lib.smgpu_get_sizes(self._h, C.byref(s)))
        return {n: getattr(s, n) for n, _ in s._fields_}

    def mesh_stats(self):
        a, b = C.c_double(), C.c_double()
        self._check(self._lib.smgpu_mesh_stats(self._h, C.byref(a), C.byref(b)))
        return a.value, b.value

    def set_params(self, p: SmoothParams):
        q = _ffi.Params(p.maxStepLength, p.relStepFrac, p.minEdgeLength, int(p.totalMinFreeze),
                        int(p.edgeAngleConstraint), int(p.faceAngleConstraint), p.minAngle, p.maxAngle)
        self._check(self._lib.smgpu_set_params(self._h, C.byref(q)))
        self.params = p

    def set_foam_variant(self, variant):
        self._check(self._lib.smgpu_set_foam_variant(self._h, {"com": 0, "org": 1}[variant]))

    def set_sync_variant(self, variant):
        self._check(self._lib.smgpu_set_sync_variant(self._h, {"master": 0, "own": 1}[variant]))

    def _layer_desc(self, lp: LayerParams, minEdgeLength: float):
        start, size, kind, sel = patch_arrays(self.mesh, lp.layerPatches)
        d = _ffi.LayerDesc()
        d.nPatches = len(start)
        d.patchStart, d.patchSize = _p(start, _ffi.c_i32p), _p(size, _ffi.c_i32p)
        d.patchKind, d.isLayerPatch = _p(kind, _ffi.c_u8p), _p(sel, _ffi.c_u8p)
        d.layerMaxBlendingFraction = lp.layerMaxBlendingFraction
        d.layerEdgeLength = minEdgeLength if lp.layerEdgeLength is None else lp.layerEdgeLength
        d.layerExpansionRatio = lp.layerExpansionRatio
        d.minLayers, d.maxLayers = lp.minLayers, lp.maxLayers
        return d, (start, size, kind, sel)

    LAYERS_HOPS_SWEEP, LAYERS_NORMALS_ACCUMULATE, LAYERS_NORMALS_FINISH, LAYERS_PROPAGATE_SWEEP, LAYERS_FINISH = range(5)
    LAYERS_F_HOPS, LAYERS_F_NORMALS_COUNT, LAYERS_F_NORMALS = range(3)
    _LAYER_FIELD_WIDTH = (1, 4, 3)

    def layers_begin(self, lp: LayerParams, minEdgeLength: float):
        d, keep = self._layer_desc(lp, minEdgeLength)
        on, it = C.c_int32(0), C.c_int32(0)
# ... 201 lines not shown
        self._check(self._lib.smgpu_enable_timing(self._h, int(on)))

    def reset_counters(self):
        self._check(self._lib.smgpu_reset_counters(self._h))

    def counters(self):
        c = _ffi.Counters()
        self._check(self._lib.smgpu_get_counters(self._h, C.byref(c)))
        return [dict(name=c.name[i].decode(), ms=c.ms[i], launches=c.launches[i], algoBytesPerLaunch=c.algoBytesPerLaunch[i],
                     algoF64OpsPerLaunch=c.algoF64OpsPerLaunch[i])
                for i in range(c.nKernels)]

    def halo_configure(self, sharedLocal, sendShared, nRecv, combOffsets, combSlots, sendA, recvA, sendF, recvF, localStats,
                       exchangeStream=None, sendL=None, recvL=None):
        keep = [np.ascontiguousarray(a, dtype=np.int32) for a in (sharedLocal, sendShared, combOffsets, combSlots)]
        d = _ffi.HaloDesc()
        d.nShared = len(keep[0]); d.sharedLocal = _p(keep[0], _ffi.c_i32p)
        d.nSend = len(keep[1]); d.sendShared = _p(keep[1], _ffi.c_i32p)
        d.nRecv = int(nRecv); d.combOffsets = _p(keep[2], _ffi.c_i32p); d.combSlots = _p(keep[3], _ffi.c_i32p)
        d.sendA, d.recvA, d.sendF, d.recvF, d.localStats = sendA, recvA, sendF, recvF, localStats
        d.sendL, d.recvL = sendL, recvL
        self._nShared = len(keep[0])
        d.useExchangeStream = 0 if exchangeStream is None else 1
        d.exchangeStream = exchangeStream or None
        self._check(self._lib.smgpu_halo_configure(self._h, C.byref(d)))

    def set_push(self, peerCount, remoteBase, myIndexAtPeer, peerRecvA, peerRecvL, peerRecvF, peerFlags, localFlags):
        n = len(peerCount)
        keep = [np.ascontiguousarray(a, dtype=np.int32) for a in (peerCount, remoteBase, myIndexAtPeer)]
        arr = lambda v: (C.c_void_p * max(n, 1))(*[C.c_void_p(int(x) if x else None) for x in v])
        ptrs = [arr(v) for v in (peerRecvA, peerRecvL, peerRecvF, peerFlags)]
        d = _ffi.PushDesc()
        d.nPeers = n
        d.peerCount, d.remoteBase, d.myIndexAtPeer = (_p(k, _ffi.c_i32p) for k in keep)
        d.peerRecvA, d.peerRecvL, d.peerRecvF, d.peerFlags = (C.cast(a, C.POINTER(C.c_void_p)) for a in ptrs)
        d.localFlags = localFlags
        self._check(self._lib.smgpu_halo_set_push(self._h, C.byref(d)))

    def clear_push(self):
        self._check(self._lib.smgpu_halo_set_push(self._h, None))

    def set_exchange_stream(self, exchangeStream):
        self._check(self._lib.smgpu_halo_set_exchange_stream(self._h, 0 if exchangeStream is None else 1, exchangeStream or None))

    def stream(self):
        out = C.c_void_p()
        self._check(self._lib.smgpu_get_stream(self._h, C.byref(out)))
        return out.value or 0

    def set_stats_history(self, ptr, capacity):
        self._check(self._lib.smgpu_halo_set_stats_history(self._h, ptr, int(capacity)))

    def iter_begin(self):
        self._check(self._lib.smgpu_iter_begin(self._h))

    def iter_interior(self):
        self._check(self._lib.smgpu_iter_interior(self._h))

    def iter_mid(self):
        self._check(self._lib.smgpu_iter_mid(self._h))

    def iter_ahead(self):
        self._check(self._lib.smgpu_iter_ahead(self._h))

    def iter_end(self):
        self._check(self._lib.smgpu_iter_end(self._h))

    def debug_walk_mode(self):
        mode, sw, cnt = C.c_int32(), C.c_int32(), C.c_int32()
        self._check(self._lib.smgpu_debug_walk_mode(self._h, C.byref(mode), C.byref(sw), C.byref(cnt)))
        self.last_active_count = cnt.value
        return mode.value, sw.value

    def debug_addressing_checksums(self):
        out = (C.c_uint64 * 64)()
        self._check(self._lib.smgpu_debug_addressing_checksums(self._h, out))
        return [int(x) for x in out][:len(TOPO_ARRAYS)]

    def debug_tile_checksums(self):
        out = (C.c_uint64 * 64)()
        self._check(self._lib.smgpu_debug_tile_checksums(self._h, out))
        return [int(x) for x in out]

    def debug_halo_mode(self):
        a, b, c = C.c_int32(), C.c_int32(), C.c_int32()
        self._check(self._lib.smgpu_debug_halo_mode(self._h, C.byref(a), C.byref(b), C.byref(c)))
        return {"multi_role": bool(a.value), "flagged": bool(b.value), "fix_inside": bool(c.value)}

    def set_device_share(self, n_engines):
        self._check(self._lib.smgpu_set_device_share(self._h, int(n_engines)))

    def debug_propose(self):
        self._check(self._lib.smgpu_debug_propose(self._h))

    def debug_field(self, name):
        n = C.c_int64()
        self._check(self._lib.smgpu_debug_get_field(self._h, name.encode(), None, C.byref(n)))
        out = np.empty(n.value, np.float64)
        self._check(self._lib.smgpu_debug_get_field(self._h, name.encode(), _p(out, _ffi.c_f64p), C.byref(n)))
        return out
```

Baseline: 12.12 billion.

## Pack per-tile topology heads into contiguous slabs for geometry and smoothing kernels

```diff
diff --git a/include/smgpu.h b/include/smgpu.h
--- a/include/smgpu.h
+++ b/include/smgpu.h
@@ -229,6 +229,7 @@
 #define SMGPU_TOPO_CHECKSUMS 64
 int smgpu_debug_addressing_checksums(smgpu_handle* h, uint64_t* out );
 int smgpu_debug_tile_checksums(smgpu_handle* h, uint64_t* out );
+int smgpu_debug_tile_head_check(smgpu_handle* h, int64_t* out );
 int smgpu_debug_halo_mode(smgpu_handle* h, int32_t* multiRole, int32_t* flagged, int32_t* fixInside);
 
 int smgpu_debug_selftest_fpexact(int32_t device, uint64_t seed, int64_t n, int64_t* mismatches);
@@ -243,6 +244,7 @@
 int smgpu_topology_get(smgpu_topology* t, const char* kind, int32_t* offsets, int32_t* values, int64_t* nnz);
 int smgpu_topology_num_edges(smgpu_topology* t, int32_t* nEdges);
 int smgpu_topology_checksums(smgpu_topology* t, uint64_t* out );
+int smgpu_topology_tile_head_check(smgpu_topology* t, const double* points, const uint8_t* isInternal, const int32_t* caps , int64_t* out );
 int smgpu_topology_destroy(smgpu_topology* t);
 
 #ifdef __cplusplus
diff --git a/smoothmesh_amd/_ffi.py b/smoothmesh_amd/_ffi.py
--- a/smoothmesh_amd/_ffi.py
+++ b/smoothmesh_amd/_ffi.py
@@ -181,6 +181,8 @@
     "smgpu_topology_checksums": (C.c_int, [C.c_void_p, C.POINTER(C.c_uint64)]),
     "smgpu_debug_addressing_checksums": (C.c_int, [C.c_void_p, C.POINTER(C.c_uint64)]),
     "smgpu_debug_tile_checksums": (C.c_int, [C.c_void_p, C.POINTER(C.c_uint64)]),
+    "smgpu_debug_tile_head_check": (C.c_int, [C.c_void_p, C.POINTER(C.c_int64)]),
+    "smgpu_topology_tile_head_check": (C.c_int, [C.c_void_p, c_f64p, C.c_void_p, c_i32p, C.POINTER(C.c_int64)]),
     "smgpu_topology_destroy": (C.c_int, [C.c_void_p]),
 }
 
diff --git a/smoothmesh_amd/csrc/kernels_tiled.hpp b/smoothmesh_amd/csrc/kernels_tiled.hpp
--- a/smoothmesh_amd/csrc/kernels_tiled.hpp
+++ b/smoothmesh_amd/csrc/kernels_tiled.hpp
@@ -1,5 +1,6 @@
 #pragma once
 #include "kernels.hpp"
+#include "tile_heads.hpp"
 
 #ifndef SMGPU_STAGGER
 #define SMGPU_STAGGER 0
@@ -28,6 +29,8 @@
     const uint8_t* tileFlags;
     const int* meta;
     int maxPoints, maxFaces;
+    const unsigned char* head;
+    int headCells;
 };
 struct GeomTileMeta { int tpOff, nPts, tfOff, nFaces, fvBase, fvWidth, cellBeg, nCells, cfBase, cfWidth, flags, pad; };
 constexpr int kGeomMetaInts = 12;
@@ -49,6 +52,7 @@
     const int* pfBase; const uint8_t* pfWidth; const uint16_t* pfEll;
     const int* meta;
     int maxCells, maxPoints, usePairShare;
+    const unsigned char* head;
 };
 
 __device__ __forceinline__ SmoothTileView pickView(bool a, const SmoothTileView& x, const SmoothTileView& y) {
@@ -56,7 +60,7 @@
 #define SMGPU_PICK(F) v.F = a ? x.F : y.F;
     SMGPU_PICK(ptOrder) SMGPU_PICK(ptBeg) SMGPU_PICK(tcOff) SMGPU_PICK(tcIds) SMGPU_PICK(tnOff) SMGPU_PICK(tnIds) SMGPU_PICK(selfLoc)
     SMGPU_PICK(pcBase) SMGPU_PICK(pcWidth) SMGPU_PICK(pcEll) SMGPU_PICK(ppBase) SMGPU_PICK(ppWidth) SMGPU_PICK(ppEll) SMGPU_PICK(pairEll)
-    SMGPU_PICK(pfBase) SMGPU_PICK(pfWidth) SMGPU_PICK(pfEll) SMGPU_PICK(meta) SMGPU_PICK(maxCells) SMGPU_PICK(maxPoints) SMGPU_PICK(usePairShare)
+    SMGPU_PICK(pfBase) SMGPU_PICK(pfWidth) SMGPU_PICK(pfEll) SMGPU_PICK(meta) SMGPU_PICK(maxCells) SMGPU_PICK(maxPoints) SMGPU_PICK(usePairShare) SMGPU_PICK(head)
 #undef SMGPU_PICK
     return v;
 }
@@ -430,6 +434,31 @@
     r.cin = geomCellLoad<T>(g, tm, tid, tflags);
     return r;
 }
+template <int T>
+__device__ __forceinline__ void geomLoadIdsHead(const unsigned char* slab, int tid, int (&id)[2]) {
+    const int* ids = reinterpret_cast<const int*>(slab);
+#pragma unroll
+    for (int u = 0; u < 2; ++u) id[u] = ids[u * T + tid];
+}
+template <int T, bool ORG>
+__device__ __forceinline__ GeomRows geomLoadRowsHead(const GeomTileView& g, const unsigned char* slab, int tid) {
+    GeomRows r;
+    const ushort4* fr = reinterpret_cast<const ushort4*>(slab + geomHeadFaceOff(T));
+#pragma unroll
+    for (int u = 0; u < 2; ++u) r.fq[u] = fr[u * T + tid];
+    const int C = g.headCells;
+    const int t = tid < C ? tid : 0;
+    r.cin.c = reinterpret_cast<const int*>(slab + geomHeadCellOff(T))[t];
+    r.cin.qa = reinterpret_cast<const ushort4*>(slab + geomHeadRowAOff(T, C))[t];
+    r.cin.qb = reinterpret_cast<const ushort4*>(slab + geomHeadRowBOff(T, C))[t];
+    r.cin.mine = false; r.preFaces = false;
+    return r;
+}
+template <bool ORG>
+__device__ __forceinline__ void geomRowsMeta(GeomRows& r, const GeomTileMeta& tm, int tid) {
+    r.preFaces = !ORG && ((unsigned)tm.flags & 1u);
+    r.cin.mine = tid < tm.nCells;
+}
 __device__ __forceinline__ void geomLoadPoints(const State& s, const int (&id)[2], V3 (&v)[2]) {
 #pragma unroll
     for (int u = 0; u < 2; ++u) v[u] = (id[u] >= 0) ? ldv(s.ptsCur, id[u]) : v3(0, 0, 0);
@@ -458,7 +487,7 @@
     for (int i = 2 * T + tid; i < nf; i += T) geomFace<ORG>(s, g, L, tm, i, tflags, wantAvg, writeFaces);
 }
 
-template <int T, bool ORG>
+template <int T, bool ORG, bool HEAD = false>
 __device__ __forceinline__ void geomTileBody(const MeshView& m, const State& s, const GeomTileView& g, int wantAvg, int writeFaces, const int* tileList,
                                              int nLaunch, int xcdMap, int deferN, int deferIter, double* deferLocal, double* deferHist, int bid, bool coh = false) {
     const int stopped = s.acc->stop;
@@ -472,10 +501,18 @@
     const GeomTileMeta tm = loadTileMeta(g, tile);
     const GeomLds L = geomLds(lds, tm);
     int id[2];
-    geomLoadIds<T>(g, tm, tid, id);
-    const GeomRows r = geomLoadRows<T, ORG>(g, tm, tid);
+    GeomRows r;
+    if (HEAD) {
+        const unsigned char* slab = g.head + geomHeadStride(T, g.headCells) * (size_t)tile;
+        geomLoadIdsHead<T>(slab, tid, id);
+        r = geomLoadRowsHead<T, ORG>(g, slab, tid);
+    } else {
+        geomLoadIds<T>(g, tm, tid, id);
+        r = geomLoadRows<T, ORG>(g, tm, tid);
+    }
     V3 v[2];
     geomLoadPoints(s, id, v);
+    if (HEAD) geomRowsMeta<ORG>(r, tm, tid);
     geomStorePoints<T>(s, g, tm, L, id, v, tid);
     if (stopped) return;
     __syncthreads();
@@ -485,11 +522,11 @@
     if (SMGPU_ABLATE & 64) return;
     geomCell<T, ORG>(s, g, L, tm, tid, (unsigned)tm.flags, r.cin, coh);
 }
-template <int T, bool ORG>
+template <int T, bool ORG, bool HEAD = false>
 __global__ void __launch_bounds__(T, (SMGPU_GEOM_WAVES * T) / 256) k_geom_tile(MeshView m, State s, GeomTileView g, int wantAvg, int writeFaces, const int* tileList,
                                                   int nLaunch, int xcdMap, int deferN, int deferIter, double* deferLocal,
                                                   double* deferHist) {
-    geomTileBody<T, ORG>(m, s, g, wantAvg, writeFaces, tileList, nLaunch, xcdMap, deferN, deferIter, deferLocal, deferHist, (int)blockIdx.x);
+    geomTileBody<T, ORG, HEAD>(m, s, g, wantAvg, writeFaces, tileList, nLaunch, xcdMap, deferN, deferIter, deferLocal, deferHist, (int)blockIdx.x);
 }
 
 struct SmoothLds { double *cx, *cy, *cz, *nx, *ny, *nz; };
@@ -536,9 +573,24 @@
     return pe[((size_t)(k >> 2) * T + tid) * 4 + (k & 3)];
 }
 struct SlotTabs { const int* slot; const int* peer; const int* dst0; const int* ndst; };
-template <int T, bool COHC = false, int SLOTS = 1>
+template <int T, bool COHC = false, int SLOTS = 1, bool HEAD = false>
 __device__ __forceinline__ SmoothRow smoothStage(const MeshView& m, const State& s, const SmoothTileView& g, const SmoothTileMeta& tm,
-                                                 const SmoothLds& L, int tid, const SlotTabs& tb = SlotTabs{nullptr, nullptr, nullptr, nullptr}) {
+                                                 const SmoothLds& L, int tid, const SlotTabs& tb = SlotTabs{nullptr, nullptr, nullptr, nullptr},
+                                                 const unsigned char* slab = nullptr) {
+    int ha[2] = {-1, -1}, hb[3] = {-1, -1, -1}, hp = -1, hself = 0;
+    ushort4 hq[6];
+    if (HEAD) {
+        const int* ic = reinterpret_cast<const int*>(slab);
+        const int* in = reinterpret_cast<const int*>(slab + smoothHeadNbrOff(T));
+#pragma unroll
+        for (int u = 0; u < 2; ++u) ha[u] = ic[u * T + tid];
+#pragma unroll
+        for (int u = 0; u < 3; ++u) hb[u] = in[u * T + tid];
+        hp = reinterpret_cast<const int*>(slab + smoothHeadPointOff(T))[tid];
+        hself = reinterpret_cast<const uint16_t*>(slab + smoothHeadSelfOff(T))[tid];
+#pragma unroll
+        for (int k = 0; k < 6; ++k) hq[k] = reinterpret_cast<const ushort4*>(slab + smoothHeadRowOff(T, k))[tid];
+    }
     SmoothRow r;
     r.peer = -1; r.dst0 = -1; r.ndst = 0;
     r.mine = tid < tm.nPts;
@@ -549,21 +601,33 @@
     const bool fast = tm.nCells <= 2 * T && tm.nNbrs <= 3 * T && r.wn4 > 0 && r.wc4 > 0;
     const ushort4 padq = make_ushort4(0xFFFF, 0xFFFF, 0xFFFF, 0xFFFF);
     if (fast) {
-        const int* ic = g.tcIds + tm.tcOff;
-        const int* in = g.tnIds + tm.tnOff;
         int a[2], b[3];
-#pragma unroll
-        for (int u = 0; u < 2; ++u) { const int i = u * T + tid; a[u] = (i < tm.nCells) ? ic[i] : -1; }
-#pragma unroll
-        for (int u = 0; u < 3; ++u) { const int i = u * T + tid; b[u] = (i < tm.nNbrs) ? in[i] : -1; }
         const int pi = tm.ptBeg + lane;
-        const int p = g.ptOrder[pi];
-        const int selfL = g.selfLoc[pi];
-        const ushort4* ppl = reinterpret_cast<const ushort4*>(g.ppEll + tm.ppBase) + lane;
-        const ushort4* pcl = reinterpret_cast<const ushort4*>(g.pcEll + tm.pcBase) + lane;
-        const ushort4 pp0 = ppl[0], pp1 = ppl[r.wn4 > 1 ? T : 0], pc0 = pcl[0], pc1 = pcl[r.wc4 > 1 ? T : 0];
-        const ushort4* pel = reinterpret_cast<const ushort4*>((g.usePairShare ? g.pairEll : g.ppEll) + tm.ppBase) + lane;
-        r.pe0 = pel[0]; r.pe1 = pel[r.wn4 > 1 ? T : 0];
+        int p, selfL;
+        ushort4 pp0, pp1, pc0, pc1;
+        if (HEAD) {
+#pragma unroll
+            for (int u = 0; u < 2; ++u) a[u] = ha[u];
+#pragma unroll
+            for (int u = 0; u < 3; ++u) b[u] = hb[u];
+            p = hp > 0 ? hp : 0;
+            selfL = hself;
+            pp0 = hq[0]; pp1 = hq[1]; pc0 = hq[2]; pc1 = hq[3]; r.pe0 = hq[4]; r.pe1 = hq[5];
+        } else {
+            const int* ic = g.tcIds + tm.tcOff;
+            const int* in = g.tnIds + tm.tnOff;
+#pragma unroll
+            for (int u = 0; u < 2; ++u) { const int i = u * T + tid; a[u] = (i < tm.nCells) ? ic[i] : -1; }
+#pragma unroll
+            for (int u = 0; u < 3; ++u) { const int i = u * T + tid; b[u] = (i < tm.nNbrs) ? in[i] : -1; }
+            p = g.ptOrder[pi];
+            selfL = g.selfLoc[pi];
+            const ushort4* ppl = reinterpret_cast<const ushort4*>(g.ppEll + tm.ppBase) + lane;
+            const ushort4* pcl = reinterpret_cast<const ushort4*>(g.pcEll + tm.pcBase) + lane;
+            pp0 = ppl[0]; pp1 = ppl[r.wn4 > 1 ? T : 0]; pc0 = pcl[0]; pc1 = pcl[r.wc4 > 1 ? T : 0];
+            const ushort4* pel = reinterpret_cast<const ushort4*>((g.usePairShare ? g.pairEll : g.ppEll) + tm.ppBase) + lane;
+            r.pe0 = pel[0]; r.pe1 = pel[r.wn4 > 1 ? T : 0];
+        }
         int slot = -1, peer = -1, dst0 = -1, ndst = 0;
         if (SLOTS == 2) { slot = tb.slot[pi]; if (tb.peer) { peer = tb.peer[pi]; dst0 = tb.dst0[pi]; ndst = tb.ndst[pi]; } }
         V3 va[2], vb[3];
@@ -738,7 +802,7 @@
     }
 }
 
-template <bool FINAL, int T>
+template <bool FINAL, int T, bool HEAD = false>
 __global__ void __launch_bounds__(T) k_smooth_tile(MeshView m, State s, Prm prm, SmoothTileView g, const int* tileList,
                                                     int nLaunch, int xcdMap) {
     const int stopped = s.acc->stop;
@@ -749,7 +813,8 @@
     const int tile = tileList ? ((const_int_ptr)tileList)[li] : li, tid = threadIdx.x;
     const SmoothTileMeta tm = loadTileMeta(g, tile);
     const SmoothLds L = smoothLds(lds, tm);
-    const SmoothRow R = smoothStage<T>(m, s, g, tm, L, tid);
+    const SmoothRow R = smoothStage<T, false, 1, HEAD>(m, s, g, tm, L, tid, SlotTabs{nullptr, nullptr, nullptr, nullptr},
+                                                      HEAD ? g.head + smoothHeadStride(T) * (size_t)tile : nullptr);
     if (stopped) return;
     __syncthreads();
     double dist = 0.0;
diff --git a/smoothmesh_amd/csrc/smgpu.hip b/smoothmesh_amd/csrc/smgpu.hip
--- a/smoothmesh_amd/csrc/smgpu.hip
+++ b/smoothmesh_amd/csrc/smgpu.hip
@@ -753,12 +753,7 @@
             if (!g.meta) {
                 const auto& gt = h->gt;
                 std::vector<int> meta((size_t)kGeomMetaInts * (size_t)gt.nTiles, 0);
-                for (int t = 0; t < gt.nTiles; ++t) {
-                    int* r = meta.data() + (size_t)kGeomMetaInts * t;
-                    r[0] = gt.tpOff[t]; r[1] = gt.tpOff[t + 1] - gt.tpOff[t]; r[2] = gt.tfOff[t]; r[3] = gt.tfOff[t + 1] - gt.tfOff[t];
-                    r[4] = gt.fvBase[t]; r[5] = gt.fvWidth[t]; r[6] = gt.cellBeg[t]; r[7] = gt.cellBeg[t + 1] - gt.cellBeg[t];
-                    r[8] = gt.cfBase[t]; r[9] = gt.cfWidth[t]; r[10] = gt.tileFlags[t];
-                }
+                geomTileMetaOf(gt, meta.data());
                 rc |= devUpload(h, &g.meta, meta);
             }
             g.maxPoints = h->gt.maxPoints; g.maxFaces = h->gt.maxFaces;
@@ -789,12 +784,7 @@
             if (!v.meta) {
                 const auto& st = h->stl;
                 std::vector<int> meta((size_t)kSmoothMetaInts * (size_t)st.nTiles, 0);
-                for (int t = 0; t < st.nTiles; ++t) {
-                    int* r = meta.data() + (size_t)kSmoothMetaInts * t;
-                    r[0] = st.ptBeg[t]; r[1] = st.ptBeg[t + 1] - st.ptBeg[t]; r[2] = st.tcOff[t]; r[3] = st.tcOff[t + 1] - st.tcOff[t];
-                    r[4] = st.tnOff[t]; r[5] = st.tnOff[t + 1] - st.tnOff[t]; r[6] = st.pcBase[t]; r[7] = st.pcWidth[t];
-                    r[8] = st.ppBase[t]; r[9] = st.ppWidth[t]; r[10] = st.pfBase[t]; r[11] = st.pfWidth[t];
-                }
+                smoothTileMetaOf(st, meta.data());
                 rc |= devUpload(h, &v.meta, meta);
             }
             v.maxCells = h->stl.maxCells; v.maxPoints = h->stl.maxPoints;
@@ -872,6 +862,24 @@
                 h->geomLds = sizeof(double) * mx;
             }
             h->smoothLds = sizeof(double) * 3 * maxTileTotal(h->stl.nTiles, {&h->stl.tcOff, &h->stl.tnOff});
+            if (envInt("SMGPU_TILE_HEAD", t.nPoints <= envInt("SMGPU_TILE_HEAD_MAX_POINTS", 4000000) ? 1 : 0) && h->gt.nTiles > 0 && h->stl.nTiles > 0) {
+                const auto t0 = std::chrono::steady_clock::now();
+                int maxCells = 1;
+                for (int ti = 0; ti < h->gt.nTiles; ++ti) maxCells = std::max(maxCells, h->gt.cellBeg[(size_t)ti + 1] - h->gt.cellBeg[(size_t)ti]);
+                const int hc = geomHeadCells(h->geomT, maxCells);
+                unsigned char *gh = nullptr, *sh = nullptr;
+                const size_t gBytes = geomHeadStride(h->geomT, hc) * (size_t)h->gt.nTiles, sBytes = smoothHeadStride(h->smoothT) * (size_t)h->stl.nTiles;
+                if (devAlloc(h, &gh, gBytes) || devAlloc(h, &sh, sBytes)) return cleanup(1);
+                const char* why = "";
+                if (packGeomHeadsOnDevice(GeomHeadSrc{g.meta, g.tpIds, g.faceVerts, g.cellOrder, g.cellFaces, h->gt.nTiles, h->geomT, hc}, gh, nullptr, &why) ||
+                    packSmoothHeadsOnDevice(SmoothHeadSrc{v.meta, v.tcIds, v.tnIds, v.ptOrder, v.selfLoc, v.ppEll, v.pcEll, v.pairEll, h->stl.nTiles, h->smoothT, v.usePairShare}, sh, nullptr, &why) ||
+                    hipStreamSynchronize(nullptr) != hipSuccess)
+                    return cleanup(fail(std::string("smgpu_create: head slabs of the tiles: ") + why));
+                g.head = gh; g.headCells = hc; v.head = sh;
+                if (envInt("SMGPU_VERBOSE", 0) >= 2)
+                    std::fprintf(stderr, "[smgpu] tile head slabs: %.1f + %.1f MB (%.1f + %.1f bytes per cell / point) packed in %.4f s\n", gBytes / 1e6, sBytes / 1e6,
+                                 (double)gBytes / std::max(1, t.nCells), (double)sBytes / std::max(1, t.nPoints), std::chrono::duration<double>(std::chrono::steady_clock::now() - t0).count());
+            }
             if (envInt("SMGPU_VERBOSE", 0))
                 std::fprintf(stderr, "[smgpu] tiles: geom T=%d n=%d LDS=%zu B (maxP %d maxF %d; staged faces x%.3f, points x%.3f of the mesh's)  smooth T=%d n=%d LDS=%zu B (maxC %d maxN %d)\n",
                              h->geomT, h->gt.nTiles, h->geomLds, g.maxPoints, g.maxFaces, (double)h->gt.tfOff.back() / std::max(1, t.nFaces),
@@ -1143,9 +1151,15 @@
         hipExtLaunchKernelGGL((k_geom_tile_bnd<T, ORG>), dim3(nBnd + tileGrid(nTiles, h->xcdMap)), dim3(T), (uint32_t)h->geomLds, h->stream, evA, evB, 0, m, s, h->gv,
                               wantAvg, h->writeFaces ? 1 : 0, tileList, nTiles, h->xcdMap, h->deferN, h->deferIter, h->deferLocal, h->deferHist, h->bv, nBnd, nNormal);
     } else {
-        ensureDynLds(k_geom_tile<T, ORG>, h->device, h->geomLds);
-        hipExtLaunchKernelGGL((k_geom_tile<T, ORG>), dim3(tileGrid(nTiles, h->xcdMap)), dim3(T), (uint32_t)h->geomLds, h->stream, evA, evB, 0, m, s, h->gv, wantAvg,
-                              h->writeFaces ? 1 : 0, tileList, nTiles, h->xcdMap, h->deferN, h->deferIter, h->deferLocal, h->deferHist);
+        if (h->gv.head) {
+            ensureDynLds(k_geom_tile<T, ORG, true>, h->device, h->geomLds);
+            hipExtLaunchKernelGGL((k_geom_tile<T, ORG, true>), dim3(tileGrid(nTiles, h->xcdMap)), dim3(T), (uint32_t)h->geomLds, h->stream, evA, evB, 0, m, s, h->gv, wantAvg,
+                                  h->writeFaces ? 1 : 0, tileList, nTiles, h->xcdMap, h->deferN, h->deferIter, h->deferLocal, h->deferHist);
+        } else {
+            ensureDynLds(k_geom_tile<T, ORG>, h->device, h->geomLds);
+            hipExtLaunchKernelGGL((k_geom_tile<T, ORG>), dim3(tileGrid(nTiles, h->xcdMap)), dim3(T), (uint32_t)h->geomLds, h->stream, evA, evB, 0, m, s, h->gv, wantAvg,
+                                  h->writeFaces ? 1 : 0, tileList, nTiles, h->xcdMap, h->deferN, h->deferIter, h->deferLocal, h->deferHist);
+        }
     }
     h->deferN = 0;
     h->deferLocal = h->deferHist = nullptr;
@@ -1158,6 +1172,12 @@
 }
 template <bool FINAL, int T>
 static void launchSmoothTile(smgpu_handle* h, const MeshView& m, const State& s, const Prm& prm, const int* tileList, int nTiles, hipEvent_t evA, hipEvent_t evB) {
+    if (h->sv.head) {
+        ensureDynLds(k_smooth_tile<FINAL, T, true>, h->device, h->smoothLds);
+        hipExtLaunchKernelGGL((k_smooth_tile<FINAL, T, true>), dim3(tileGrid(nTiles, h->xcdMap)), dim3(T), (uint32_t)h->smoothLds, h->stream, evA, evB, 0, m, s, prm, h->sv,
+                              tileList, nTiles, h->xcdMap);
+        return;
+    }
     ensureDynLds(k_smooth_tile<FINAL, T>, h->device, h->smoothLds);
     hipExtLaunchKernelGGL((k_smooth_tile<FINAL, T>), dim3(tileGrid(nTiles, h->xcdMap)), dim3(T), (uint32_t)h->smoothLds, h->stream, evA, evB, 0, m, s, prm, h->sv,
                           tileList, nTiles, h->xcdMap);
@@ -3389,6 +3409,9 @@
             dev(h->sv.selfLoc, (size_t)h->mv.nPoints * 2) || dev(h->sv.pcEll, nPc * 2) || dev(h->sv.ppEll, nPp * 2) || dev(h->sv.pairEll, nPp * 2) || dev(h->sv.pfEll, nPfE * 2) ||
             dev(h->sv.meta, (size_t)nS * kSmoothMetaInts * 4)) return 1;
     }
+    if (h->gv.head && h->sv.head) {
+        if (dev(h->gv.head, geomHeadStride(h->geomT, h->gv.headCells) * (size_t)nT) || dev(h->sv.head, smoothHeadStride(h->smoothT) * (size_t)h->stl.nTiles)) return 1;
+    }
     if (h->useFilter && h->ev.meta) {
         const EdgeTiles& et = h->etl;
         const int nE = et.nTiles;
@@ -3404,6 +3427,55 @@
     return 0;
 }
 
+int smgpu_debug_tile_head_check(smgpu_handle* h, int64_t* out) {
+    if (!h || !out) return fail("null argument");
+    for (int i = 0; i < 4; ++i) out[i] = 0;
+    if (!h->useTiles || !h->gv.head || !h->sv.head) return 0;
+    HIP_OK(hipSetDevice(h->device));
+    HIP_OK(hipDeviceSynchronize());
+    const GeomTiles& gt = h->gt;
+    const SmoothTiles& st = h->stl;
+    const int nT = gt.nTiles, nS = st.nTiles;
+    auto get = [&](auto& v, const void* p, size_t n) -> int {
+        v.resize(std::max<size_t>(n, 1));
+        if (n) HIP_OK(hipMemcpy(v.data(), p, n * sizeof(v[0]), hipMemcpyDeviceToHost));
+        return 0;
+    };
+    auto differing = [](const std::vector<unsigned char>& a, const std::vector<unsigned char>& b) { int64_t n = 0; for (size_t i = 0; i < a.size(); ++i) n += a[i] != b[i]; return n; };
+    out[0] = 1;
+    {
+        const size_t nFv = nT ? (size_t)gt.fvBase[(size_t)nT - 1] + (size_t)(gt.tfOff[(size_t)nT] - gt.tfOff[(size_t)nT - 1]) * gt.fvWidth[(size_t)nT - 1] : 0;
+        const size_t nCf = nT ? (size_t)gt.cfBase[(size_t)nT - 1] + (size_t)gt.cfWidth[(size_t)nT - 1] * (size_t)gt.threads : 0;
+        std::vector<int> meta, tpIds, cellOrder;
+        std::vector<uint16_t> faceVerts, cellFaces;
+        std::vector<unsigned char> devHead, hostHead;
+        const size_t bytes = geomHeadStride(h->geomT, h->gv.headCells) * (size_t)nT;
+        if (get(meta, h->gv.meta, (size_t)nT * kGeomMetaInts) || get(tpIds, h->gv.tpIds, (size_t)gt.tpOff.back()) || get(cellOrder, h->gv.cellOrder, (size_t)h->mv.nCells) ||
+            get(faceVerts, h->gv.faceVerts, nFv) || get(cellFaces, h->gv.cellFaces, nCf) || get(devHead, h->gv.head, bytes)) return 1;
+        hostHead.assign(devHead.size(), 0);
+        packGeomHeads(GeomHeadSrc{meta.data(), tpIds.data(), faceVerts.data(), cellOrder.data(), cellFaces.data(), nT, h->geomT, h->gv.headCells}, hostHead.data());
+        out[1] = (int64_t)bytes;
+        out[2] = differing(devHead, hostHead);
+    }
+    {
+        const size_t nPc = nS ? (size_t)st.pcBase[(size_t)nS - 1] + (size_t)st.pcWidth[(size_t)nS - 1] * (size_t)st.threads : 0;
+        const size_t nPp = nS ? (size_t)st.ppBase[(size_t)nS - 1] + (size_t)st.ppWidth[(size_t)nS - 1] * (size_t)st.threads : 0;
+        std::vector<int> meta, tcIds, tnIds, ptOrder;
+        std::vector<uint16_t> selfLoc, ppEll, pcEll, pairEll;
+        std::vector<unsigned char> devHead, hostHead;
+        const size_t bytes = smoothHeadStride(h->smoothT) * (size_t)nS;
+        if (get(meta, h->sv.meta, (size_t)nS * kSmoothMetaInts) || get(tcIds, h->sv.tcIds, (size_t)st.tcOff.back()) || get(tnIds, h->sv.tnIds, (size_t)st.tnOff.back()) ||
+            get(ptOrder, h->sv.ptOrder, (size_t)h->mv.nPoints) || get(selfLoc, h->sv.selfLoc, (size_t)h->mv.nPoints) || get(ppEll, h->sv.ppEll, nPp) || get(pcEll, h->sv.pcEll, nPc) ||
+            get(pairEll, h->sv.pairEll, nPp) || get(devHead, h->sv.head, bytes)) return 1;
+        hostHead.assign(devHead.size(), 0);
+        packSmoothHeads(SmoothHeadSrc{meta.data(), tcIds.data(), tnIds.data(), ptOrder.data(), selfLoc.data(), ppEll.data(), pcEll.data(), pairEll.data(), nS, h->smoothT, h->sv.usePairShare},
+                        hostHead.data());
+        out[1] += (int64_t)bytes;
+        out[3] = differing(devHead, hostHead);
+    }
+    return 0;
+}
+
 int smgpu_debug_addressing_checksums(smgpu_handle* h, uint64_t* out) {
     if (!h || !out) return fail("null argument");
     if (ensureHostLists(h, 3)) return 1;
@@ -3437,6 +3509,36 @@
     topoChecksums(t->t, out);
     return 0;
 }
+int smgpu_topology_tile_head_check(smgpu_topology* tp, const double* points, const uint8_t* isInternal, const int32_t* caps, int64_t* out) {
+    if (!tp || !points || !isInternal || !caps || !out) return fail("null argument");
+    const Topology& t = tp->t;
+    const int T = caps[0];
+    if (T != 64 && T != 128 && T != 256) return fail("smgpu_topology_tile_head_check: 64, 128 or 256 threads");
+    GeomTiles gt;
+    SmoothTiles st;
+    const int geomCells = caps[1] > 0 ? caps[1] : T / 2;
+    std::string e = gt.build(t, points, true, T, geomCells, caps[2] > 0 ? caps[2] : std::min(6 * geomCells, 1400), caps[3] > 0 ? caps[3] : std::min(4 * geomCells, 1400),
+                             (caps[2] > 0 || caps[3] > 0) ? 0x7fffffff : defaultGeomCapWeighted(T), SMGPU_GEOM_AOS ? kGF : 6);
+    if (e.empty()) e = st.build(t, points, isInternal, true, T, caps[4] > 0 ? caps[4] : std::min(2 * T, 1500), caps[5] > 0 ? caps[5] : std::min(3 * T, 1500), nullptr, nullptr,
+                                (caps[4] > 0 || caps[5] > 0) ? 0x7fffffff : defaultSmoothCapTotal(T));
+    if (!e.empty()) return fail("smgpu_topology_tile_head_check: " + e);
+    int maxCells = 1;
+    for (int ti = 0; ti < gt.nTiles; ++ti) maxCells = std::max(maxCells, gt.cellBeg[(size_t)ti + 1] - gt.cellBeg[(size_t)ti]);
+    const int hc = geomHeadCells(T, maxCells), usePairShare = t.maxPointPoints <= 16 ? 1 : 0;
+    std::vector<int> gm((size_t)kTileMetaInts * std::max(gt.nTiles, 1)), sm((size_t)kTileMetaInts * std::max(st.nTiles, 1));
+    geomTileMetaOf(gt, gm.data());
+    smoothTileMetaOf(st, sm.data());
+    std::vector<unsigned char> gh(geomHeadStride(T, hc) * (size_t)gt.nTiles + 1, 0xA5), sh(smoothHeadStride(T) * (size_t)st.nTiles + 1, 0xA5);
+    packGeomHeads(GeomHeadSrc{gm.data(), gt.tpIds.data(), gt.faceVerts.data(), gt.order.data(), gt.cellFaces.data(), gt.nTiles, T, hc}, gh.data());
+    packSmoothHeads(SmoothHeadSrc{sm.data(), st.tcIds.data(), st.tnIds.data(), st.order.data(), st.selfLoc.data(), st.ppEll.data(), st.pcEll.data(), st.pairEll.data(), st.nTiles, T, usePairShare},
+                    sh.data());
+    const HeadCheck a = checkGeomHeads(gt, hc, gh.data()), b = checkSmoothHeads(st, usePairShare, sh.data());
+    out[0] = gt.nTiles; out[1] = a.live; out[2] = a.pads; out[3] = a.wrong; out[4] = a.beyond;
+    out[5] = st.nTiles; out[6] = b.live; out[7] = b.pads; out[8] = b.wrong; out[9] = b.beyond;
+    out[10] = (gh.back() == 0xA5 && sh.back() == 0xA5) ? 0 : 1;
+    out[11] = (int64_t)(gh.size() + sh.size() - 2);
+    return 0;
+}
 int smgpu_topology_num_edges(smgpu_topology* t, int32_t* nEdges) {
     if (!t || !nEdges) return fail("null argument");
     *nEdges = t->t.nEdges;
diff --git a/smoothmesh_amd/csrc/tile_heads.hpp b/smoothmesh_amd/csrc/tile_heads.hpp
--- /dev/null
+++ b/smoothmesh_amd/csrc/tile_heads.hpp
@@ -0,0 +1,102 @@
+#pragma once
+#include <cstddef>
+#include <cstdint>
+
+#if defined(__HIP__)
+#define SMGPU_HEAD_HD __host__ __device__
+#else
+#define SMGPU_HEAD_HD
+#endif
+
+namespace smgpu {
+
+constexpr int kTileMetaInts = 12;
+
+SMGPU_HEAD_HD inline int geomHeadCells(int threads, int capCells) { const int c = ((capCells < 1 ? 1 : capCells) + 63) & ~63; return c < threads ? c : threads; }
+SMGPU_HEAD_HD inline size_t geomHeadFaceOff(int T) { return (size_t)8 * T; }
+SMGPU_HEAD_HD inline size_t geomHeadCellOff(int T) { return (size_t)24 * T; }
+SMGPU_HEAD_HD inline size_t geomHeadRowAOff(int T, int C) { return (size_t)24 * T + (size_t)4 * C; }
+SMGPU_HEAD_HD inline size_t geomHeadRowBOff(int T, int C) { return (size_t)24 * T + (size_t)12 * C; }
+SMGPU_HEAD_HD inline size_t geomHeadStride(int T, int C) { return (size_t)24 * T + (size_t)20 * C; }
+
+SMGPU_HEAD_HD inline size_t smoothHeadNbrOff(int T) { return (size_t)8 * T; }
+SMGPU_HEAD_HD inline size_t smoothHeadPointOff(int T) { return (size_t)20 * T; }
+SMGPU_HEAD_HD inline size_t smoothHeadSelfOff(int T) { return (size_t)24 * T; }
+SMGPU_HEAD_HD inline size_t smoothHeadRowOff(int T, int k ) { return (size_t)26 * T + (size_t)8 * T * k; }
+SMGPU_HEAD_HD inline size_t smoothHeadStride(int T) { return (size_t)74 * T; }
+
+struct GeomHeadSrc {
+    const int* meta; const int* tpIds; const uint16_t* faceVerts; const int* cellOrder; const uint16_t* cellFaces;
+    int nTiles, threads, cells;
+};
+struct SmoothHeadSrc {
+    const int* meta; const int* tcIds; const int* tnIds; const int* ptOrder; const uint16_t* selfLoc;
+    const uint16_t* ppEll; const uint16_t* pcEll; const uint16_t* pairEll;
+    int nTiles, threads, usePairShare;
+};
+
+struct HeadRow { uint16_t x, y, z, w; };
+SMGPU_HEAD_HD inline HeadRow headRowOf(const uint16_t* p) { HeadRow r; r.x = p[0]; r.y = p[1]; r.z = p[2]; r.w = p[3]; return r; }
+SMGPU_HEAD_HD inline HeadRow headRowPad() { HeadRow r; r.x = r.y = r.z = r.w = 0xFFFFu; return r; }
+
+SMGPU_HEAD_HD inline void packGeomHeadTile(const GeomHeadSrc& s, int tile, unsigned char* head, int first, int step) {
+    const int T = s.threads, C = s.cells;
+    const int* m = s.meta + (size_t)kTileMetaInts * tile;
+    const int tpOff = m[0], nPts = m[1], nFaces = m[3], fvBase = m[4], fvWidth = m[5], cellBeg = m[6], nCells = m[7], cfBase = m[8], cfWidth = m[9], flags = m[10];
+    unsigned char* slab = head + geomHeadStride(T, C) * (size_t)tile;
+    int* pointId = reinterpret_cast<int*>(slab);
+    HeadRow* faceRow = reinterpret_cast<HeadRow*>(slab + geomHeadFaceOff(T));
+    int* cellId = reinterpret_cast<int*>(slab + geomHeadCellOff(T));
+    HeadRow* rowA = reinterpret_cast<HeadRow*>(slab + geomHeadRowAOff(T, C));
+    HeadRow* rowB = reinterpret_cast<HeadRow*>(slab + geomHeadRowBOff(T, C));
+    const bool quads = (flags & 1) && fvWidth == 4, six = (flags & 2) && cfWidth >= 8;
+    for (int i = first; i < 2 * T; i += step) {
+        pointId[i] = i < nPts ? s.tpIds[(size_t)tpOff + i] : -1;
+        faceRow[i] = (quads && i < nFaces) ? headRowOf(s.faceVerts + (size_t)fvBase + (size_t)4 * i) : headRowPad();
+    }
+    for (int t = first; t < C; t += step) {
+        const bool mine = t < nCells;
+        cellId[t] = mine ? s.cellOrder[(size_t)cellBeg + t] : -1;
+        rowA[t] = (mine && six) ? headRowOf(s.cellFaces + (size_t)cfBase + (size_t)4 * t) : headRowPad();
+        rowB[t] = (mine && six) ? headRowOf(s.cellFaces + (size_t)cfBase + (size_t)4 * (T + t)) : headRowPad();
+    }
+}
+SMGPU_HEAD_HD inline void packSmoothHeadTile(const SmoothHeadSrc& s, int tile, unsigned char* head, int first, int step) {
+    const int T = s.threads;
+    const int* m = s.meta + (size_t)kTileMetaInts * tile;
+    const int ptBeg = m[0], nPts = m[1], tcOff = m[2], nCells = m[3], tnOff = m[4], nNbrs = m[5], pcBase = m[6], pcWidth = m[7], ppBase = m[8], ppWidth = m[9];
+    unsigned char* slab = head + smoothHeadStride(T) * (size_t)tile;
+    int* cellId = reinterpret_cast<int*>(slab);
+    int* nbrId = reinterpret_cast<int*>(slab + smoothHeadNbrOff(T));
+    int* pointId = reinterpret_cast<int*>(slab + smoothHeadPointOff(T));
+    uint16_t* selfLoc = reinterpret_cast<uint16_t*>(slab + smoothHeadSelfOff(T));
+    for (int i = first; i < 2 * T; i += step) cellId[i] = i < nCells ? s.tcIds[(size_t)tcOff + i] : -1;
+    for (int i = first; i < 3 * T; i += step) nbrId[i] = i < nNbrs ? s.tnIds[(size_t)tnOff + i] : -1;
+    for (int t = first; t < T; t += step) {
+        const bool mine = t < nPts;
+        pointId[t] = mine ? s.ptOrder[(size_t)ptBeg + t] : -1;
+        selfLoc[t] = mine ? s.selfLoc[(size_t)ptBeg + t] : (uint16_t)0xFFFFu;
+        for (int k = 0; k < 6; ++k) {
+            const uint16_t* ell = k < 2 ? s.ppEll : (k < 4 ? s.pcEll : s.pairEll);
+            const int base = (k == 2 || k == 3) ? pcBase : ppBase, width = (k == 2 || k == 3) ? pcWidth : ppWidth, chunk = k & 1;
+            const bool live = mine && width >= 4 * (chunk + 1) && (k < 4 || s.usePairShare);
+            reinterpret_cast<HeadRow*>(slab + smoothHeadRowOff(T, k))[t] = live ? headRowOf(ell + (size_t)base + (size_t)4 * ((size_t)chunk * T + t)) : headRowPad();
+        }
+    }
+}
+
+void packGeomHeads(const GeomHeadSrc& s, unsigned char* out);
+void packSmoothHeads(const SmoothHeadSrc& s, unsigned char* out);
+int packGeomHeadsOnDevice(const GeomHeadSrc& s, unsigned char* out, void* stream, const char** why);
+int packSmoothHeadsOnDevice(const SmoothHeadSrc& s, unsigned char* out, void* stream, const char** why);
+
+
+struct GeomTiles;
+struct SmoothTiles;
+void geomTileMetaOf(const GeomTiles& gt, int* meta);
+void smoothTileMetaOf(const SmoothTiles& st, int* meta);
+struct HeadCheck { long long live = 0, pads = 0, wrong = 0, beyond = 0; };
+HeadCheck checkGeomHeads(const GeomTiles& gt, int cells, const unsigned char* head);
+HeadCheck checkSmoothHeads(const SmoothTiles& st, int usePairShare, const unsigned char* head);
+
+}
diff --git a/smoothmesh_amd/csrc/tiles.cpp b/smoothmesh_amd/csrc/tiles.cpp
--- a/smoothmesh_amd/csrc/tiles.cpp
+++ b/smoothmesh_amd/csrc/tiles.cpp
@@ -5,6 +5,7 @@
 #include <chrono>
 #include <cstdio>
 #include <cstdlib>
+#include <cstring>
 
 namespace smgpu {
 
@@ -716,4 +717,91 @@
     return "";
 }
 
-}
+void packGeomHeads(const GeomHeadSrc& s, unsigned char* out) {
+    for (int t = 0; t < s.nTiles; ++t) packGeomHeadTile(s, t, out, 0, 1);
+}
+void packSmoothHeads(const SmoothHeadSrc& s, unsigned char* out) {
+    for (int t = 0; t < s.nTiles; ++t) packSmoothHeadTile(s, t, out, 0, 1);
+}
+
+void geomTileMetaOf(const GeomTiles& gt, int* meta) {
+    for (int t = 0; t < gt.nTiles; ++t) {
+        int* r = meta + (size_t)kTileMetaInts * t;
+        r[0] = gt.tpOff[t]; r[1] = gt.tpOff[t + 1] - gt.tpOff[t]; r[2] = gt.tfOff[t]; r[3] = gt.tfOff[t + 1] - gt.tfOff[t];
+        r[4] = gt.fvBase[t]; r[5] = gt.fvWidth[t]; r[6] = gt.cellBeg[t]; r[7] = gt.cellBeg[t + 1] - gt.cellBeg[t];
+        r[8] = gt.cfBase[t]; r[9] = gt.cfWidth[t]; r[10] = gt.tileFlags[t]; r[11] = 0;
+    }
+}
+void smoothTileMetaOf(const SmoothTiles& st, int* meta) {
+    for (int t = 0; t < st.nTiles; ++t) {
+        int* r = meta + (size_t)kTileMetaInts * t;
+        r[0] = st.ptBeg[t]; r[1] = st.ptBeg[t + 1] - st.ptBeg[t]; r[2] = st.tcOff[t]; r[3] = st.tcOff[t + 1] - st.tcOff[t];
+        r[4] = st.tnOff[t]; r[5] = st.tnOff[t + 1] - st.tnOff[t]; r[6] = st.pcBase[t]; r[7] = st.pcWidth[t];
+        r[8] = st.ppBase[t]; r[9] = st.ppWidth[t]; r[10] = st.pfBase[t]; r[11] = st.pfWidth[t];
+    }
+}
+
+namespace {
+struct HeadTally {
+    HeadCheck c;
+    void id(int got, bool live, int want) { (live ? c.live : c.pads)++; if (got != (live ? want : -1)) ++c.wrong; }
+    void u16(uint16_t got, bool live, uint16_t want) { (live ? c.live : c.pads)++; if (got != (live ? want : kEllPad)) ++c.wrong; }
+    void row(const unsigned char* got, bool live, const uint16_t* want) {
+        uint16_t g[4];
+        std::memcpy(g, got, 8);
+        for (int k = 0; k < 4; ++k) u16(g[k], live, live ? want[k] : kEllPad);
+    }
+};
+int intAt(const unsigned char* p, size_t i) { int v; std::memcpy(&v, p + 4 * i, 4); return v; }
+}
+
+HeadCheck checkGeomHeads(const GeomTiles& gt, int cells, const unsigned char* head) {
+    HeadTally y;
+    const int T = gt.threads, C = cells;
+    for (int t = 0; t < gt.nTiles; ++t) {
+        const unsigned char* slab = head + geomHeadStride(T, C) * (size_t)t;
+        const int nPts = gt.tpOff[t + 1] - gt.tpOff[t], nFaces = gt.tfOff[t + 1] - gt.tfOff[t], nCells = gt.cellBeg[t + 1] - gt.cellBeg[t];
+        const bool quads = gt.tileFlags[t] & 1, six = gt.tileFlags[t] & 2;
+        if (nPts > 2 * T || nFaces > 2 * T) ++y.c.beyond;
+        for (int i = 0; i < 2 * T; ++i) {
+            y.id(intAt(slab, (size_t)i), i < nPts, i < nPts ? gt.tpIds[(size_t)gt.tpOff[t] + i] : 0);
+            y.row(slab + geomHeadFaceOff(T) + 8 * (size_t)i, quads && i < nFaces, gt.faceVerts.data() + (size_t)gt.fvBase[t] + (size_t)gt.fvWidth[t] * i);
+        }
+        for (int k = 0; k < C; ++k) {
+            const bool mine = k < nCells;
+            y.id(intAt(slab + geomHeadCellOff(T), (size_t)k), mine, mine ? gt.order[(size_t)gt.cellBeg[t] + k] : 0);
+            y.row(slab + geomHeadRowAOff(T, C) + 8 * (size_t)k, mine && six, gt.cellFaces.data() + (size_t)gt.cfBase[t] + ((size_t)0 * T + k) * 4);
+            y.row(slab + geomHeadRowBOff(T, C) + 8 * (size_t)k, mine && six, gt.cellFaces.data() + (size_t)gt.cfBase[t] + ((size_t)1 * T + k) * 4);
+        }
+    }
+    return y.c;
+}
+HeadCheck checkSmoothHeads(const SmoothTiles& st, int usePairShare, const unsigned char* head) {
+    HeadTally y;
+    const int T = st.threads;
+    for (int t = 0; t < st.nTiles; ++t) {
+        const unsigned char* slab = head + smoothHeadStride(T) * (size_t)t;
+        const int nPts = st.ptBeg[t + 1] - st.ptBeg[t], nCells = st.tcOff[t + 1] - st.tcOff[t], nNbrs = st.tnOff[t + 1] - st.tnOff[t];
+        if (nCells > 2 * T || nNbrs > 3 * T) ++y.c.beyond;
+        for (int i = 0; i < 2 * T; ++i) y.id(intAt(slab, (size_t)i), i < nCells, i < nCells ? st.tcIds[(size_t)st.tcOff[t] + i] : 0);
+        for (int i = 0; i < 3 * T; ++i) y.id(intAt(slab + smoothHeadNbrOff(T), (size_t)i), i < nNbrs, i < nNbrs ? st.tnIds[(size_t)st.tnOff[t] + i] : 0);
+        for (int k = 0; k < T; ++k) {
+            const bool mine = k < nPts;
+            const size_t pos = (size_t)st.ptBeg[t] + k;
+            y.id(intAt(slab + smoothHeadPointOff(T), (size_t)k), mine, mine ? st.order[pos] : 0);
+            uint16_t sl;
+            std::memcpy(&sl, slab + smoothHeadSelfOff(T) + 2 * (size_t)k, 2);
+            y.u16(sl, mine, mine ? st.selfLoc[pos] : kEllPad);
+            for (int chunk = 0; chunk < 2; ++chunk) {
+                const size_t ppAt = (size_t)st.ppBase[t] + ((size_t)chunk * T + k) * 4, pcAt = (size_t)st.pcBase[t] + ((size_t)chunk * T + k) * 4;
+                const bool pp = mine && st.ppWidth[t] > 4 * chunk, pc = mine && st.pcWidth[t] > 4 * chunk;
+                y.row(slab + smoothHeadRowOff(T, 0 + chunk) + 8 * (size_t)k, pp, st.ppEll.data() + ppAt);
+                y.row(slab + smoothHeadRowOff(T, 2 + chunk) + 8 * (size_t)k, pc, st.pcEll.data() + pcAt);
+                y.row(slab + smoothHeadRowOff(T, 4 + chunk) + 8 * (size_t)k, pp && usePairShare, st.pairEll.data() + ppAt);
+            }
+        }
+    }
+    return y.c;
+}
+
+}
diff --git a/smoothmesh_amd/csrc/tiles.hpp b/smoothmesh_amd/csrc/tiles.hpp
--- a/smoothmesh_amd/csrc/tiles.hpp
+++ b/smoothmesh_amd/csrc/tiles.hpp
@@ -3,6 +3,7 @@
 #include <string>
 #include <vector>
 
+#include "tile_heads.hpp"
 #include "topology.hpp"
 
 namespace smgpu {
diff --git a/smoothmesh_amd/csrc/tiles_dev.hip b/smoothmesh_amd/csrc/tiles_dev.hip
--- a/smoothmesh_amd/csrc/tiles_dev.hip
+++ b/smoothmesh_amd/csrc/tiles_dev.hip
@@ -817,4 +817,23 @@
     return 0;
 }
 
-}
+namespace {
+__global__ void __launch_bounds__(kT) k_tl_geomHead(GeomHeadSrc s, unsigned char* head) { packGeomHeadTile(s, (int)blockIdx.x, head, (int)threadIdx.x, kT); }
+__global__ void __launch_bounds__(kT) k_tl_smoothHead(SmoothHeadSrc s, unsigned char* head) { packSmoothHeadTile(s, (int)blockIdx.x, head, (int)threadIdx.x, kT); }
+}
+int packGeomHeadsOnDevice(const GeomHeadSrc& s, unsigned char* out, void* stream, const char** why) {
+    if (s.nTiles <= 0) return 0;
+    hipLaunchKernelGGL(k_tl_geomHead, dim3(s.nTiles), dim3(kT), 0, (hipStream_t)stream, s, out);
+    const hipError_t e = hipGetLastError();
+    if (e != hipSuccess) { if (why) *why = hipGetErrorString(e); return 2; }
+    return 0;
+}
+int packSmoothHeadsOnDevice(const SmoothHeadSrc& s, unsigned char* out, void* stream, const char** why) {
+    if (s.nTiles <= 0) return 0;
+    hipLaunchKernelGGL(k_tl_smoothHead, dim3(s.nTiles), dim3(kT), 0, (hipStream_t)stream, s, out);
+    const hipError_t e = hipGetLastError();
+    if (e != hipSuccess) { if (why) *why = hipGetErrorString(e); return 2; }
+    return 0;
+}
+
+}
diff --git a/smoothmesh_amd/engine.py b/smoothmesh_amd/engine.py
--- a/smoothmesh_amd/engine.py
+++ b/smoothmesh_amd/engine.py
@@ -174,6 +174,16 @@
             raise SmgpuError(self._lib.smgpu_last_error().decode())
         return [int(x) for x in out][:len(TOPO_ARRAYS)]
 
+    def tile_head_check(self, is_internal, threads=256, geom_cells=0, geom_cap_points=0, geom_cap_faces=0, smooth_cap_cells=0, smooth_cap_nbrs=0):
+        ip = np.ascontiguousarray(is_internal, dtype=np.uint8)
+        caps = np.array([threads, geom_cells, geom_cap_points, geom_cap_faces, smooth_cap_cells, smooth_cap_nbrs], np.int32)
+        out = (C.c_int64 * 12)()
+        if self._lib.smgpu_topology_tile_head_check(self._h, _p(self._keep["pts"], _ffi.c_f64p), ip.ctypes.data_as(C.c_void_p), _p(caps, _ffi.c_i32p), out):
+            raise SmgpuError(self._lib.smgpu_last_error().decode())
+        keys = ("tiles", "live", "pads", "wrong", "beyond")
+        return {"geometry": dict(zip(keys, [int(x) for x in out[0:5]])), "smoothing": dict(zip(keys, [int(x) for x in out[5:10]])),
+                "overrun": int(out[10]), "bytes": int(out[11])}
+
     def close(self):
         if self._h:
             self._lib.smgpu_topology_destroy(self._h)
@@ -541,6 +551,11 @@
         self._check(self._lib.smgpu_debug_tile_checksums(self._h, out))
         return [int(x) for x in out]
 
+    def debug_tile_head_check(self):
+        out = (C.c_int64 * 4)()
+        self._check(self._lib.smgpu_debug_tile_head_check(self._h, out))
+        return {"in_use": bool(out[0]), "bytes": int(out[1]), "geometry_differ": int(out[2]), "smoothing_differ": int(out[3])}
+
     def debug_halo_mode(self):
         a, b, c = C.c_int32(), C.c_int32(), C.c_int32()
         self._check(self._lib.smgpu_debug_halo_mode(self._h, C.byref(a), C.byref(b), C.byref(c)))
```

New measurement: 12.25 billion, median of 2. No clear change (+1.1%).
